# wangxiaohit/GNNPN-SC

Hardware: AMD Instinct MI355X
Metric: service-composition problems/sec (ML+2PN inference) (higher is better)
Workload: dtype f32-split3xf16 (f32 operands and results; recurrent W_hh.h products: fp32 operands split exactly into 3 x f16, six f16-matrix-core products per term, f32 accumulate; everything else f32 arithmetic)

## Files before the change

gnnpn-sc_amd/csrc/api.hip:

```cpp
#include "common.h"
#include <string.h>
#include <mutex>
#include "lstm_shared.h"
#include "decode_shared.h"
#include "coop_common.h"

thread_local char g_gnnpn_err[256] = "";

thread_local int64_t g_gnnpn_last_units = 0;
extern "C" int64_t gnnpn_last_launch_units(void) { return g_gnnpn_last_units; }

thread_local int g_gnnpn_lds_footprint_kb = 0;
extern "C" int gnnpn_lds_footprint_kb(int kb) {
    const int prev = g_gnnpn_lds_footprint_kb;
    if (kb >= 0 && kb <= 160) g_gnnpn_lds_footprint_kb = kb;
    return prev;
}
unsigned gnnpn_front_lds_pad(const void* func) { return gnnpn_lds_padding(func, g_gnnpn_lds_footprint_kb); }

extern "C" int gnnpn_abi_version(void) { return GNNPN_ABI_VERSION; }
extern "C" const char* gnnpn_last_error(void) { return g_gnnpn_err; }

static int g_lstm_ablate = 0;
int gnnpn_option_lstm_ablate() { return g_lstm_ablate; }

unsigned* gnnpn_cu_seat_table() {
    static unsigned* table[64] = {nullptr};
    static std::mutex mu;
    int dev = 0;
    if (hipGetDevice(&dev) != hipSuccess || dev < 0 || dev >= 64) return nullptr;
    std::lock_guard<std::mutex> lock(mu);
    if (!table[dev]) {
        unsigned* p = nullptr;
        if (hipMalloc(&p, COOP_SEAT_TABLE_WORDS * sizeof(unsigned)) != hipSuccess) return nullptr;
        if (hipMemset(p, 0, COOP_SEAT_TABLE_WORDS * sizeof(unsigned)) != hipSuccess) return nullptr;
        if (hipDeviceSynchronize() != hipSuccess) return nullptr;
        table[dev] = p;
    }
    return table[dev];
}

extern "C" int gnnpn_coop_reset_staffing(void) {
    unsigned* p = gnnpn_cu_seat_table();
    if (!p) GNNPN_FAIL(GNNPN_E_LAUNCH, "coop_reset_staffing: no seat table");
    if (hipDeviceSynchronize() != hipSuccess || hipMemset(p + COOP_STAFFING_WORD, 0, sizeof(unsigned)) != hipSuccess)
        GNNPN_FAIL(GNNPN_E_LAUNCH, "coop_reset_staffing: memset failed");
    return GNNPN_OK;
}

extern "C" int gnnpn_coop_staffing_count(void) {
    unsigned* p = gnnpn_cu_seat_table();
    unsigned v = 0;
    if (!p || hipDeviceSynchronize() != hipSuccess || hipMemcpy(&v, p + COOP_STAFFING_WORD, sizeof(v), hipMemcpyDeviceToHost) != hipSuccess) return -1;
    return (int)v;
}

extern "C" int gnnpn_set_option(const char* name, int value) {
    if (!name) GNNPN_FAIL(GNNPN_E_ARG, "set_option: null name");
    if (!strcmp(name, "lstm_ablate")) {
        GNNPN_REQUIRE(value >= 0 && (value & 128) == 0, "set_option: lstm_ablate bit 7 is gnnpn_launch_opts_t.write_through now");
        g_lstm_ablate = value;
        return GNNPN_OK;
    }
    GNNPN_FAIL(GNNPN_E_ARG, "set_option: unknown option '%s' (impl / lds_kb / write_through are gnnpn_launch_opts_t fields)", name);
}

__global__ void cell_activations_kernel(const float* __restrict__ x, float* __restrict__ sig, float* __restrict__ th,
                                        int64_t n) {
    const int64_t i = blockIdx.x * (int64_t)blockDim.x + threadIdx.x;
    if (i < n) {
        sig[i] = cell_sigmoid(x[i]);
        th[i] = cell_tanh(x[i]);
    }
}

extern "C" int gnnpn_debug_cell_activations(const float* x, float* sig, float* th, int64_t n, void* stream) {
    GNNPN_REQUIRE(x && sig && th && n >= 0, "debug_cell_activations: bad argument");
    if (n == 0) return GNNPN_OK;
    hipLaunchKernelGGL(cell_activations_kernel, dim3((unsigned)((n + 255) / 256)), dim3(256), 0, (hipStream_t)stream,
                       x, sig, th, n);
    GNNPN_CHECK_LAUNCH("debug_cell_activations");
    return GNNPN_OK;
}

namespace {
__global__ void gate_wait_kernel(const unsigned* __restrict__ flag, unsigned expect, unsigned long long ticks) {
    const unsigned long long t0 = __builtin_amdgcn_s_memrealtime();
    while (__hip_atomic_load(flag, __ATOMIC_RELAXED, __HIP_MEMORY_SCOPE_SYSTEM) != expect &&
           __builtin_amdgcn_s_memrealtime() - t0 < ticks)
        __builtin_amdgcn_s_sleep(20);
}
}

extern "C" int gnnpn_gate_wait(const void* flag, uint32_t expect, int32_t timeout_us, void* stream) {
    GNNPN_REQUIRE(flag && timeout_us >= 0 && timeout_us <= 100000, "gate_wait: a flag in pinned host (or device) memory, a time-out of at most 0.1 s");
    GNNPN_REQUIRE(gnnpn_aligned(flag, 4), "gate_wait: the flag must be 4-byte aligned");
    hipLaunchKernelGGL(gate_wait_kernel, dim3(1), dim3(64), 0, static_cast<hipStream_t>(stream), static_cast<const unsigned*>(flag), expect,
                       (unsigned long long)timeout_us * 100ull);
    GNNPN_CHECK_LAUNCH("gate_wait");
    return GNNPN_OK;
}
```

gnnpn-sc_amd/csrc/coop_common.h:

```cpp
#pragma once
#include "common.h"
#include "lstm_shared.h"

typedef float f32x4 __attribute__((ext_vector_type(4)));
typedef unsigned long long u64;

__device__ __forceinline__ void granule_store(u64* p, unsigned tag, float v) {
    __hip_atomic_store(p, ((u64)tag << 32) | __float_as_uint(v), __ATOMIC_RELAXED,
                       __HIP_MEMORY_SCOPE_AGENT);
}

typedef unsigned u32x4 __attribute__((ext_vector_type(4)));
#define GNNPN_LD2(dst, voff, sbase, off) "global_load_dwordx4 " dst ", " voff ", " sbase " offset:" off " sc1\n\t"
__device__ __forceinline__ const u64* uniform_ptr(const u64* p) {
    const unsigned long long v = (unsigned long long)p;
    const unsigned lo = __builtin_amdgcn_readfirstlane((unsigned)v), hi = __builtin_amdgcn_readfirstlane((unsigned)(v >> 32));
    return reinterpret_cast<const u64*>(((unsigned long long)hi << 32) | lo);
}
__device__ __forceinline__ void granule_reload2_x8_masked(u32x4 (&v)[8], const u64* base, unsigned voff, unsigned long long lanes) {
    const u64* q = base + 512;
    unsigned long long saved;
    asm volatile("s_and_saveexec_b64 %8, %12\n\t"
                 GNNPN_LD2("%0", "%9", "%10", "0") GNNPN_LD2("%1", "%9", "%10", "1024") GNNPN_LD2("%2", "%9", "%10", "2048")
                 GNNPN_LD2("%3", "%9", "%10", "3072") GNNPN_LD2("%4", "%9", "%11", "0") GNNPN_LD2("%5", "%9", "%11", "1024")
                 GNNPN_LD2("%6", "%9", "%11", "2048") GNNPN_LD2("%7", "%9", "%11", "3072")
                 "s_waitcnt vmcnt(0)\n\t"
                 "s_mov_b64 exec, %8"
                 : "+v"(v[0]), "+v"(v[1]), "+v"(v[2]), "+v"(v[3]), "+v"(v[4]), "+v"(v[5]), "+v"(v[6]), "+v"(v[7]), "=&s"(saved)
                 : "v"(voff), "s"(base), "s"(q), "s"(lanes)
                 : "memory", "scc");
}
__device__ __forceinline__ void granule_load2_x8_x4(u32x4 (&v)[8], u32x4 (&w)[4], const u64* base, const u64* pbase, unsigned voff) {
    const u64* q = base + 512;
    asm volatile(GNNPN_LD2("%0", "%12", "%13", "0") GNNPN_LD2("%1", "%12", "%13", "1024") GNNPN_LD2("%2", "%12", "%13", "2048")
                 GNNPN_LD2("%3", "%12", "%13", "3072") GNNPN_LD2("%4", "%12", "%14", "0") GNNPN_LD2("%5", "%12", "%14", "1024")
                 GNNPN_LD2("%6", "%12", "%14", "2048") GNNPN_LD2("%7", "%12", "%14", "3072")
                 GNNPN_LD2("%8", "%12", "%15", "0") GNNPN_LD2("%9", "%12", "%15", "1024") GNNPN_LD2("%10", "%12", "%15", "2048")
                 GNNPN_LD2("%11", "%12", "%15", "3072")
                 "s_waitcnt vmcnt(0)"
                 : "=&v"(v[0]), "=&v"(v[1]), "=&v"(v[2]), "=&v"(v[3]), "=&v"(v[4]), "=&v"(v[5]), "=&v"(v[6]), "=&v"(v[7]),
                   "=&v"(w[0]), "=&v"(w[1]), "=&v"(w[2]), "=&v"(w[3])
                 : "v"(voff), "s"(base), "s"(q), "s"(pbase)
                 : "memory");
}

__device__ __forceinline__ void granule_load2_x8_x4_lat(u32x4 (&v)[8], u32x4 (&w)[4], u64& lat, const u64* base, const u64* pbase,
                                                        const u64* lbase, unsigned voff) {
    const u64* q = base + 512;
    asm volatile(GNNPN_LD2("%0", "%13", "%15", "0") GNNPN_LD2("%1", "%13", "%15", "1024") GNNPN_LD2("%2", "%13", "%15", "2048")
                 GNNPN_LD2("%3", "%13", "%15", "3072") GNNPN_LD2("%4", "%13", "%16", "0") GNNPN_LD2("%5", "%13", "%16", "1024")
                 GNNPN_LD2("%6", "%13", "%16", "2048") GNNPN_LD2("%7", "%13", "%16", "3072")
                 GNNPN_LD2("%8", "%13", "%17", "0") GNNPN_LD2("%9", "%13", "%17", "1024") GNNPN_LD2("%10", "%13", "%17", "2048")
                 GNNPN_LD2("%11", "%13", "%17", "3072")
                 "global_load_dwordx2 %12, %14, %18 sc1\n\t"
                 "s_waitcnt vmcnt(0)"
                 : "=&v"(v[0]), "=&v"(v[1]), "=&v"(v[2]), "=&v"(v[3]), "=&v"(v[4]), "=&v"(v[5]), "=&v"(v[6]), "=&v"(v[7]),
                   "=&v"(w[0]), "=&v"(w[1]), "=&v"(w[2]), "=&v"(w[3]), "=&v"(lat)
                 : "v"(voff), "v"(voff >> 1), "s"(base), "s"(q), "s"(pbase), "s"(lbase)
                 : "memory");
}

constexpr int COOP_STAFFING_WORD = 8 * 256 + 8;
__device__ __forceinline__ void coop_raise(unsigned* err, unsigned* sticky, unsigned code, unsigned* seats = nullptr) {
    atomicOr(err, code);
    if (sticky) atomicOr(sticky, code);
    if (seats && atomicCAS(err + 4, 1u, 2u) == 1u) atomicSub(seats + COOP_STAFFING_WORD, 1u);
}

constexpr int COOP_STATUS_BYTES = 16384;
constexpr unsigned COOP_LDS_UNITS = 640;
constexpr int COOP_XCD_STRIDE = 32;
constexpr int COOP_XCDCNT_OFFSET = 12288;
constexpr int COOP_ARRIVE_OFFSET = 13312;
constexpr int COOP_PLACED_OFFSET = 14336;
constexpr int COOP_CLAIM_OFFSET = 2048;
constexpr int COOP_TAKEN_OFFSET = 10240;
constexpr int COOP_OVERREAD_BYTES = 4096;
constexpr int COOP_OVERSUB = 3;
constexpr unsigned COOP_SURPLUS_WAIT_TICKS = 1600;
constexpr unsigned COOP_RESERVE_WAIT_TICKS = 200000;

__device__ __forceinline__ unsigned xcc_id() {
    return __builtin_amdgcn_s_getreg(20 | (0 << 6) | (3 << 11)) & 0xfu;
}

__device__ __forceinline__ void granule_store_l2_bits(u64* p, u64 g) {
    asm volatile("global_store_dwordx2 %0, %1, off" ::"v"(p), "v"(g) : "memory");
}
__device__ __forceinline__ void granule_store_l2(u64* p, unsigned tag, float v) {
    granule_store_l2_bits(p, ((u64)tag << 32) | __float_as_uint(v));
}
__device__ __forceinline__ void granule_publish(u64* p, unsigned tag, float v, bool same_xcd) {
    if (same_xcd) granule_store_l2(p, tag, v);
    else granule_store(p, tag, v);
}

namespace {
__global__ __launch_bounds__(256) void coop_zero_kernel(unsigned long long* __restrict__ p, size_t n8, unsigned* __restrict__ sticky,
                                                        int word, unsigned expected, int skip_zeroing) {
    if (sticky && blockIdx.x == 0 && threadIdx.x == 0) atomicAdd(sticky + word, expected);
    if (skip_zeroing) return;
    for (size_t i = blockIdx.x * (size_t)blockDim.x + threadIdx.x; i < n8; i += (size_t)gridDim.x * blockDim.x)
        __hip_atomic_store(p + i, 0ull, __ATOMIC_RELAXED, __HIP_MEMORY_SCOPE_AGENT);
}
}
inline hipError_t coop_zero_workspace(void* workspace, size_t bytes, hipStream_t s, unsigned* sticky, int word, unsigned expected,
                                      bool skip_zeroing = false) {
    const size_t n8 = bytes / 8;
    unsigned blocks = skip_zeroing ? 1u : (unsigned)((n8 + 255) / 256);
    if (blocks > 2048) blocks = 2048;
    hipLaunchKernelGGL(coop_zero_kernel, dim3(blocks), dim3(256), 0, s, static_cast<unsigned long long*>(workspace), n8, sticky, word,
                       expected, skip_zeroing ? 1 : 0);
    return hipGetLastError();
}

constexpr int COOP_G = 8, COOP_ROWS = 16, COOP_H = 256;

struct CoopLaunch {
    int n_tiles, gpx, groups, groups_per_net;
    unsigned* status;
    char* buffers;
    unsigned* seats;
};

template <typename Need>
inline int coop_begin(const char* who, int n_nets, int32_t rows, Need need, int expected_word, const CoopOpts& opts,
                      void* workspace, int64_t workspace_bytes, hipStream_t s, CoopLaunch& L) {
    int dev = 0, n_cu = 0;
    if (hipGetDevice(&dev) != hipSuccess ||
        hipDeviceGetAttribute(&n_cu, hipDeviceAttributeMultiprocessorCount, dev) != hipSuccess)
        GNNPN_FAIL(GNNPN_E_LAUNCH, "%s: cannot query the device", who);
    L.n_tiles = (rows + COOP_ROWS - 1) / COOP_ROWS;
    L.gpx = n_cu / (8 * COOP_G);
    if (L.gpx > 8) L.gpx = 8;
    while (L.gpx > 1 && (L.gpx - 1) * 8 >= n_nets * L.n_tiles) --L.gpx;
    if (L.gpx < 1 || n_cu < 256)
        GNNPN_FAIL(GNNPN_E_UNSUP, "%s: device has %d CUs, the cooperative form is built for 8 XCDs x 32 CUs", who, n_cu);
    L.groups = L.gpx * 8;
    if (L.groups < n_nets) GNNPN_FAIL(GNNPN_E_UNSUP, "%s: %d groups for %d nets", who, L.groups, n_nets);
    L.groups_per_net = L.groups / n_nets;
    const int64_t bytes = need(L.groups);
    if (!workspace || workspace_bytes < bytes || !gnnpn_aligned(workspace, 256))
        GNNPN_FAIL(GNNPN_E_ARG, "%s: workspace of %lld B (256-B aligned) required", who, (long long)bytes);
    L.seats = gnnpn_cu_seat_table();
    if (!L.seats) GNNPN_FAIL(GNNPN_E_LAUNCH, "%s: cannot allocate the seat table", who);
    const unsigned units = (unsigned)(COOP_G * n_nets * L.n_tiles);
    if (coop_zero_workspace(workspace, (size_t)bytes, s, opts.sticky, expected_word, units, (gnnpn_option_lstm_ablate() & 0x2000) != 0) !=
        hipSuccess)
        GNNPN_FAIL(GNNPN_E_LAUNCH, "%s: workspace memset failed", who);
    g_gnnpn_last_units = opts.sticky ? (int64_t)units : 0;
    L.status = static_cast<unsigned*>(workspace);
    L.buffers = static_cast<char*>(workspace) + COOP_STATUS_BYTES;
    return GNNPN_OK;
}

struct DecodeWorkspace {
    int64_t h_bytes, p_bytes, l_bytes;
    int64_t total() const { return COOP_STATUS_BYTES + h_bytes + p_bytes + l_bytes + COOP_OVERREAD_BYTES; }
};
inline DecodeWorkspace decode_workspace(int64_t groups, int64_t rows, int32_t T, int32_t K, int64_t xp_granules) {
    const int64_t tiles = (rows + COOP_ROWS - 1) / COOP_ROWS;
    return {groups * 2 * COOP_ROWS * COOP_H * 8, groups * 2 * xp_granules * 8, tiles * T * COOP_ROWS * (int64_t)K * 8};
}
__device__ __forceinline__ void coop_note_finished(unsigned* sticky, int word, unsigned tiles_done) {
    if (sticky && tiles_done) atomicAdd(sticky + word, tiles_done);
}

__device__ __forceinline__ void coop_note_staffed(unsigned* status, unsigned* count_xcc, unsigned target, unsigned* seats) {
    if (atomicAdd(count_xcc, 1u) + 1u == target && atomicAdd(status + 5, 1u) + 1u == 8u && atomicExch(status + 4, 2u) == 1u)
        atomicSub(seats + COOP_STAFFING_WORD, 1u);
}
template <int G>
__device__ __forceinline__ bool coop_place(unsigned* status, int gpx, int* slot, int& group, int& member, unsigned* seats,
                                           bool paired_start = false, unsigned* sticky = nullptr) {
    if (threadIdx.x < 64) {
        const int lane = threadIdx.x;
        const unsigned xcc = xcc_id();
        unsigned* count = status + COOP_XCDCNT_OFFSET / 4;
        unsigned* arrive = status + COOP_ARRIVE_OFFSET / 4;
        unsigned* taken = status + COOP_TAKEN_OFFSET / 4 + xcc * 64;
        const unsigned target = (unsigned)(gpx * G);
        auto staffed = [&]() {
            unsigned v = 0;
            if (lane == 0) v = __hip_atomic_load(status + 5, __ATOMIC_RELAXED, __HIP_MEMORY_SCOPE_AGENT);
            return __shfl(v, 0, 64) >= 8u;
        };
        int g = -1, m = 0;
#ifndef GNNPN_COOP_NO_ENTRY_ACQUIRE
        __builtin_amdgcn_fence(__ATOMIC_ACQUIRE, "agent");
#endif
        const unsigned hw = __builtin_amdgcn_s_getreg(4 | (0 << 6) | (31 << 11));
        const unsigned key = (xcc << 8) | ((hw >> 8) & 0xffu);
        unsigned* staffing = seats + COOP_STAFFING_WORD;
        const unsigned* word = lane < 8 ? count + COOP_XCD_STRIDE * lane : lane == 9 ? status + 4 : seats + key;
        unsigned got = 0;
        if (lane < 12 && lane != 8 && lane != 10) got = __hip_atomic_load(word, __ATOMIC_RELAXED, __HIP_MEMORY_SCOPE_AGENT);
        if (lane == 8) got = atomicAdd(arrive + COOP_XCD_STRIDE * xcc, 1u);
        const bool staffed_at_entry = __all(lane >= 8 || got >= target);
        unsigned arrival = __shfl(got, 8, 64);
        const bool marked = __shfl(got, 9, 64) != 0u;
        const unsigned seat_seen = __shfl(got, 11, 64);
        if (lane == 0) {
            if (arrival == 0u && !marked && atomicCAS(status + 4, 0u, 1u) == 0u) atomicAdd(staffing, 1u);
            if (arrival >= gridDim.x / 8 || (staffed_at_entry && arrival < target)) coop_raise(status, sticky, 8u);
        }
        if (!staffed_at_entry) {
            if (lane == 0) {
                atomicAdd(status + COOP_CLAIM_OFFSET / 4 + key, 1u);
                const unsigned la = __builtin_amdgcn_s_getreg(6 | (0 << 6) | (31 << 11));
                const unsigned lds_base = la & 0xfffu, lds_size = (la >> 12) & 0xfffu;
                const bool badly_placed = lds_base != 0u && lds_base < lds_size && lds_base + 2u * lds_size > COOP_LDS_UNITS;
                bool another_staffing = false;
                if (badly_placed && !paired_start) {
                    if (atomicCAS(status + 4, 0u, 1u) == 0u) atomicAdd(staffing, 1u);
                    another_staffing = __hip_atomic_load(staffing, __ATOMIC_RELAXED, __HIP_MEMORY_SCOPE_AGENT) > 1u;
                }
                const bool fragments = (paired_start || another_staffing) && badly_placed;
                const bool reserve_arrival = arrival + target >= gridDim.x / 8;
                if (fragments && !reserve_arrival) {
                    atomicAdd(status + 3, 1u);
                    if (sticky) atomicAdd(sticky + GNNPN_STATUS_DECLINED_SEATS, 1u);
                    g = -2;
                } else if (!fragments) {
                    unsigned s = seat_seen;
                    if (s == 0u) {
                        if (atomicCAS(seats + key, 0u, 0xffffffffu) == 0u) {
                            s = atomicAdd(seats + 8 * 256 + xcc, 1u) + 1u;
                            __hip_atomic_store(seats + key, s, __ATOMIC_RELAXED, __HIP_MEMORY_SCOPE_AGENT);
                        } else {
                            s = 0xffffffffu;
                        }
                    }
                    for (unsigned spin = 0; s == 0xffffffffu && spin < 100000u; ++spin)
                        s = __hip_atomic_load(seats + key, __ATOMIC_RELAXED, __HIP_MEMORY_SCOPE_AGENT);
                    const unsigned seat = s - 1u;
                    if (seat < target && atomicCAS(taken + seat, 0u, 1u) == 0u) {
                        g = (int)xcc * gpx + (int)(seat / G);
                        m = (int)(seat % G);
                        coop_note_staffed(status, count + COOP_XCD_STRIDE * xcc, target, seats);
                    }
                }
            }
            g = __shfl(g, 0, 64);
            m = __shfl(m, 0, 64);
            arrival = __shfl(arrival, 0, 64);
            if (g == -2) {
                g = -1;
            } else if (g < 0) {
                const unsigned per_xcd = gridDim.x / 8;
                const bool reserve = arrival + target >= per_xcd;
                const unsigned long long patience = reserve ? COOP_RESERVE_WAIT_TICKS : COOP_SURPLUS_WAIT_TICKS;
                const unsigned long long t0 = __builtin_amdgcn_s_memrealtime();
                bool done = staffed();
                while (!done && __builtin_amdgcn_s_memrealtime() - t0 < patience) {
                    __builtin_amdgcn_s_sleep(8);
                    done = staffed();
                }
                if (!done && reserve) {
                    if (lane == 0) {
                        for (unsigned seat = 0; seat < target && g < 0; ++seat) {
                            if (atomicCAS(taken + seat, 0u, 1u) == 0u) {
                                g = (int)xcc * gpx + (int)(seat / G);
                                m = (int)(seat % G);
                                coop_note_staffed(status, count + COOP_XCD_STRIDE * xcc, target, seats);
                                atomicAdd(status + 2, 1u);
                                if (sticky) atomicAdd(sticky + GNNPN_STATUS_OFF_CANONICAL_SEATS, 1u);
                            }
                        }
                    }
                    g = __shfl(g, 0, 64);
                    m = __shfl(m, 0, 64);
                }
            }
        }
        if (lane == 0) {
            slot[0] = g;
            slot[1] = m;
        }
    }
    __syncthreads();
    group = slot[0];
    member = slot[1];
    return group >= 0;
}

__device__ __forceinline__ float swap8(float v) {
    return __int_as_float(__builtin_amdgcn_update_dpp(0, __float_as_int(v), 0x128 , 0xF, 0xF, false));
}

__device__ __forceinline__ u64 phase_stamp() {
    u64 t;
    __builtin_amdgcn_sched_barrier(0);
    asm volatile("s_memtime %0\n\ts_waitcnt lgkmcnt(0)" : "=s"(t)::"memory");
    __builtin_amdgcn_sched_barrier(0);
    return t;
}

constexpr int LDT = 260;
__device__ __forceinline__ int ht_index(int row, int unit) { return row * LDT + (unit & 3) * 64 + (unit >> 2); }

struct NoHook {
    __device__ __forceinline__ void operator()() const {}
};
template <int LD, int CH = 16, bool KQ = false, typename Mid = NoHook>
__device__ __forceinline__ void mfma_chain_pair(const float* src, int c, int kq, const float (&w0)[64],
                                                const float (&w1)[64], f32x4& acc0, f32x4& acc1, Mid mid = Mid()) {
    const float* base = KQ ? src + c * LD + kq * 64 : src + c * LD + kq;
    const float4* base4 = reinterpret_cast<const float4*>(base);
    float a[2][CH];
    auto fetch = [&](int ch, float (&dst)[CH]) {
        if constexpr (KQ) {
#pragma unroll
            for (int q = 0; q < CH / 4; ++q) {
                const float4 v = base4[(CH / 4) * ch + q];
                dst[4 * q] = v.x; dst[4 * q + 1] = v.y; dst[4 * q + 2] = v.z; dst[4 * q + 3] = v.w;
            }
        } else {
#pragma unroll
            for (int i = 0; i < CH; ++i) dst[i] = base[4 * (CH * ch + i)];
        }
    };
    fetch(0, a[0]);
#pragma unroll
    for (int ch = 0; ch < 64 / CH; ++ch) {
        if (ch < 64 / CH - 1) fetch(ch + 1, a[(ch + 1) & 1]);
        __builtin_amdgcn_sched_barrier(0);
#pragma unroll
        for (int i = 0; i < CH; ++i) {
            acc0 = __builtin_amdgcn_mfma_f32_16x16x4f32(a[ch & 1][i], w0[CH * ch + i], acc0, 0, 0, 0);
            acc1 = __builtin_amdgcn_mfma_f32_16x16x4f32(a[ch & 1][i], w1[CH * ch + i], acc1, 0, 0, 0);
        }
        __builtin_amdgcn_sched_barrier(0);
        if (ch == 64 / CH / 2 - 1) mid();
    }
}

typedef _Float16 f16x8 __attribute__((ext_vector_type(8)));
constexpr int LDH16 = 264;
constexpr int SPLIT_TILE = 16 * LDH16;
constexpr float SPLIT_SCALE = 2048.0f, SPLIT_INV = 1.0f / 2048.0f;
constexpr float SPLIT_H_SCALE = 32768.0f, SPLIT_H_INV = 1.0f / 32768.0f;

__device__ __forceinline__ void split3(float xs, _Float16& p0, _Float16& p1, _Float16& p2) {
    p0 = (_Float16)xs;
    const float r1 = __fmul_rn(__fsub_rn(xs, (float)p0), SPLIT_SCALE);
    p1 = (_Float16)r1;
    p2 = (_Float16)__fmul_rn(__fsub_rn(r1, (float)p1), SPLIT_SCALE);
}
__device__ __forceinline__ unsigned short f16_bits(_Float16 v) { return __builtin_bit_cast(unsigned short, v); }

__device__ __forceinline__ unsigned split_tag16(unsigned tag) { return 0x8000u | (tag & 0x7fffu); }
__device__ __forceinline__ u64 split_granule(unsigned tag, float h) {
    _Float16 p0, p1, p2;
    split3(__fmul_rn(h, SPLIT_H_SCALE), p0, p1, p2);
    const unsigned d0 = (unsigned)f16_bits(p0) | (split_tag16(tag) << 16);
    const unsigned d1 = (unsigned)f16_bits(p1) | ((unsigned)f16_bits(p2) << 16);
    return ((u64)d1 << 32) | d0;
}
__device__ __forceinline__ void split_granule_store(u64* p, unsigned tag, float h, bool same_xcd) {
    const u64 g = split_granule(tag, h);
    if (same_xcd) granule_store_l2_bits(p, g);
    else __hip_atomic_store(p, g, __ATOMIC_RELAXED, __HIP_MEMORY_SCOPE_AGENT);
}
__device__ __forceinline__ bool split_pair_tagged(u32x4 v, unsigned tag) {
    const unsigned t = split_tag16(tag);
    return __builtin_amdgcn_perm(v.z, v.x, 0x07060302u) == (t | (t << 16));
}
__device__ __forceinline__ void split_pair_to_lds(_Float16* at, u32x4 v) {
    unsigned* d = reinterpret_cast<unsigned*>(at);
    d[0] = __builtin_amdgcn_perm(v.z, v.x, 0x05040100u);
    d[SPLIT_TILE / 2] = __builtin_amdgcn_perm(v.w, v.y, 0x05040100u);
    d[SPLIT_TILE] = __builtin_amdgcn_perm(v.w, v.y, 0x07060302u);
}
__device__ __forceinline__ void split_store(_Float16* at, float h) {
    _Float16 p0, p1, p2;
    split3(__fmul_rn(h, SPLIT_H_SCALE), p0, p1, p2);
    at[0] = p0;
    at[SPLIT_TILE] = p1;
    at[2 * SPLIT_TILE] = p2;
}

constexpr int SPLIT_WT_DWORDS = 4 * 8 * 64 * 4;
template <int HD>
__device__ __forceinline__ float split_weights(const float* __restrict__ Wp, int gate, int u, int kq, f16x8 (&w0)[8],
                                               f16x8 (&w1)[8], unsigned* wt) {
    float m = 0.0f;
#pragma unroll
    for (int kk = 0; kk < 8; ++kk)
#pragma unroll
        for (int j = 0; j < 8; ++j)
            m = fmaxf(m, fabsf(Wp[((size_t)((8 * kk + 2 * kq + (j >> 2)) * 4 + gate) * HD + u) * 4 + (j & 3)]));
    m = fmaxf(m, __shfl_xor(m, 16, 64));
    m = fmaxf(m, __shfl_xor(m, 32, 64));
    int e = 0;
    if (m > 0.0f && m < 3.0e38f) (void)frexpf(m, &e);
    int s = m > 0.0f ? 15 - e : 0;
    s = s > 96 ? 96 : (s < -96 ? -96 : s);
    const float up = ldexpf(1.0f, s);
#pragma unroll
    for (int kk = 0; kk < 8; ++kk) {
        unsigned bytes[2] = {0u, 0u};
#pragma unroll
        for (int j = 0; j < 8; ++j) {
            const float w = Wp[((size_t)((8 * kk + 2 * kq + (j >> 2)) * 4 + gate) * HD + u) * 4 + (j & 3)];
            _Float16 p0, p1, p2;
            split3(__fmul_rn(w, up), p0, p1, p2);
            w0[kk][j] = p0;
            w1[kk][j] = p1;
            bytes[j >> 2] |= (unsigned)(f16_bits(p2) >> 8) << (8 * (j & 3));
        }
        wt[4 * 64 * kk] = bytes[0];
        wt[4 * 64 * kk + 1] = bytes[1];
    }
    return ldexpf(1.0f, -(15 + s));
}
constexpr int SPLIT_PACK_U4_PER_MEMBER = 2 * 2 * 8 * 256 + 8 * 256 + 2 * 256 / 4;
constexpr int SPLIT_PACK_MEMBERS = 8;
__device__ __forceinline__ void load_split_weights(const uint4* __restrict__ pk, int tid, f16x8 (&w0)[2][8], f16x8 (&w1)[2][8],
                                                   unsigned* wt_lane, float (&inv)[2]) {
#pragma unroll
    for (int tl = 0; tl < 2; ++tl)
#pragma unroll
        for (int kk = 0; kk < 8; ++kk) {
            w0[tl][kk] = __builtin_bit_cast(f16x8, pk[((tl * 2 + 0) * 8 + kk) * 256 + tid]);
            w1[tl][kk] = __builtin_bit_cast(f16x8, pk[((tl * 2 + 1) * 8 + kk) * 256 + tid]);
        }
#pragma unroll
    for (int kk = 0; kk < 8; ++kk) *reinterpret_cast<uint4*>(wt_lane + 4 * 64 * kk) = pk[8192 + kk * 256 + tid];
    const float* fi = reinterpret_cast<const float*>(pk + 10240);
    inv[0] = fi[tid];
    inv[1] = fi[256 + tid];
}

__device__ __forceinline__ f16x8 split_expand(unsigned lo, unsigned hi) {
    const u32x4 r = {__builtin_amdgcn_perm(0u, lo, 0x010c000cu), __builtin_amdgcn_perm(0u, lo, 0x030c020cu),
                     __builtin_amdgcn_perm(0u, hi, 0x010c000cu), __builtin_amdgcn_perm(0u, hi, 0x030c020cu)};
    return __builtin_bit_cast(f16x8, r);
}
template <typename Mid = NoHook>
__device__ __forceinline__ void split_chain(const _Float16* base, const f16x8 (&w0)[2][8], const f16x8 (&w1)[2][8],
                                            const unsigned* wt, const float (&inv)[2], f32x4 (&acc)[2], Mid mid = Mid()) {
    constexpr int NT = 2;
    f32x4 a0[NT], a0b[NT], a1[NT], a2[NT];
#pragma unroll
    for (int n = 0; n < NT; ++n) a0[n] = a0b[n] = a1[n] = a2[n] = f32x4{0.f, 0.f, 0.f, 0.f};
    f16x8 h0[2];
    h0[0] = *reinterpret_cast<const f16x8*>(base);
    f16x8 h1 = *reinterpret_cast<const f16x8*>(base + SPLIT_TILE);
    f16x8 h2 = *reinterpret_cast<const f16x8*>(base + 2 * SPLIT_TILE);
    u32x4 t = *reinterpret_cast<const u32x4*>(wt);
#define GNNPN_FENCE __builtin_amdgcn_sched_barrier(0)
#pragma unroll
    for (int kk = 0; kk < 8; ++kk) {
        const int nx = 32 * (kk + 1), cur = kk & 1;
        u32x4 e0, e1;
        if (kk < 7) h0[cur ^ 1] = *reinterpret_cast<const f16x8*>(base + nx);
        GNNPN_FENCE;
        a2[0] = __builtin_amdgcn_mfma_f32_16x16x32_f16(h1, w1[0][kk], a2[0], 0, 0, 0);
        e0.x = __builtin_amdgcn_perm(0u, t.x, 0x010c000cu);
        e0.y = __builtin_amdgcn_perm(0u, t.x, 0x030c020cu);
        GNNPN_FENCE;
        a2[1] = __builtin_amdgcn_mfma_f32_16x16x32_f16(h1, w1[1][kk], a2[1], 0, 0, 0);
        e0.z = __builtin_amdgcn_perm(0u, t.y, 0x010c000cu);
        e0.w = __builtin_amdgcn_perm(0u, t.y, 0x030c020cu);
        GNNPN_FENCE;
        a1[0] = __builtin_amdgcn_mfma_f32_16x16x32_f16(h1, w0[0][kk], a1[0], 0, 0, 0);
        e1.x = __builtin_amdgcn_perm(0u, t.z, 0x010c000cu);
        e1.y = __builtin_amdgcn_perm(0u, t.z, 0x030c020cu);
        GNNPN_FENCE;
        a1[1] = __builtin_amdgcn_mfma_f32_16x16x32_f16(h1, w0[1][kk], a1[1], 0, 0, 0);
        e1.z = __builtin_amdgcn_perm(0u, t.w, 0x010c000cu);
        e1.w = __builtin_amdgcn_perm(0u, t.w, 0x030c020cu);
        GNNPN_FENCE;
        if (kk < 7) {
            h1 = *reinterpret_cast<const f16x8*>(base + SPLIT_TILE + nx);
            t = *reinterpret_cast<const u32x4*>(wt + 4 * 64 * (kk + 1));
        }
        a2[0] = __builtin_amdgcn_mfma_f32_16x16x32_f16(h0[cur], __builtin_bit_cast(f16x8, e0), a2[0], 0, 0, 0);
        GNNPN_FENCE;
        a2[1] = __builtin_amdgcn_mfma_f32_16x16x32_f16(h0[cur], __builtin_bit_cast(f16x8, e1), a2[1], 0, 0, 0);
        GNNPN_FENCE;
        if (kk < 4) a0[0] = __builtin_amdgcn_mfma_f32_16x16x32_f16(h0[cur], w0[0][kk], a0[0], 0, 0, 0);
        else a0b[0] = __builtin_amdgcn_mfma_f32_16x16x32_f16(h0[cur], w0[0][kk], a0b[0], 0, 0, 0);
        GNNPN_FENCE;
        if (kk < 4) a0[1] = __builtin_amdgcn_mfma_f32_16x16x32_f16(h0[cur], w0[1][kk], a0[1], 0, 0, 0);
        else a0b[1] = __builtin_amdgcn_mfma_f32_16x16x32_f16(h0[cur], w0[1][kk], a0b[1], 0, 0, 0);
        GNNPN_FENCE;
        a2[0] = __builtin_amdgcn_mfma_f32_16x16x32_f16(h2, w0[0][kk], a2[0], 0, 0, 0);
        GNNPN_FENCE;
        a2[1] = __builtin_amdgcn_mfma_f32_16x16x32_f16(h2, w0[1][kk], a2[1], 0, 0, 0);
        GNNPN_FENCE;
        if (kk < 7) h2 = *reinterpret_cast<const f16x8*>(base + 2 * SPLIT_TILE + nx);
        a1[0] = __builtin_amdgcn_mfma_f32_16x16x32_f16(h0[cur], w1[0][kk], a1[0], 0, 0, 0);
        GNNPN_FENCE;
        a1[1] = __builtin_amdgcn_mfma_f32_16x16x32_f16(h0[cur], w1[1][kk], a1[1], 0, 0, 0);
        GNNPN_FENCE;
        if (kk == 3) mid();
    }
#undef GNNPN_FENCE
#pragma unroll
    for (int n = 0; n < NT; ++n)
#pragma unroll
        for (int r = 0; r < 4; ++r)
            acc[n][r] = __fmul_rn(fmaf(fmaf(a2[n][r], SPLIT_INV, a1[n][r]), SPLIT_INV, __fadd_rn(a0[n][r], a0b[n][r])), inv[n]);
}

__device__ __forceinline__ void cell_update_split(const f32x2 (&g0)[2], const f32x2 (&g1)[2], bool lo_half, f32x2& cst, f32x2& h) {
    f32x2 a0[2], a1[2];
#pragma unroll
    for (int q = 0; q < 2; ++q) {
        a0[q] = cell_act2(g0[q], false);
        a1[q] = cell_act2(g1[q], lo_half);
    }
    const f32x2 s0 = lo_half ? a0[1] : a0[0], s1 = lo_half ? a1[1] : a1[0];
    const f32x2 t0 = {swap8(s0.x), swap8(s0.y)}, t1 = {swap8(s1.x), swap8(s1.y)};
    const f32x2 ig = lo_half ? a0[0] : t0, gg = lo_half ? a1[0] : t1;
    const f32x2 fg = lo_half ? t0 : a0[1], og = lo_half ? t1 : a1[1];
    cst = fg * cst + ig * gg;
    h = og * cell_act2(cst, true);
}
```

gnnpn-sc_amd/csrc/decode_lean.hip:

```cpp
#include "common.h"
#include "recurrent.h"
#include "decode_shared.h"
#include "coop_common.h"
#include "lstm_shared.h"

namespace {
constexpr int H = COOP_H;
constexpr int G = COOP_G;
constexpr int ROWS = COOP_ROWS;
constexpr int UNITS = H / G;
constexpr int KW = 16;
constexpr unsigned SPIN_LIMIT = 400000;
constexpr int XP_GRANULES = ROWS * KW * G;

typedef unsigned u32x2 __attribute__((ext_vector_type(2)));
constexpr int AUX_SC1 = 16;


__device__ __forceinline__ __amdgpu_buffer_rsrc_t make_rsrc(const void* p, unsigned bytes) {
    return __builtin_amdgcn_make_buffer_rsrc(const_cast<void*>(p), 0, (int)bytes, 0x00020000);
}
__device__ __forceinline__ float dpp_ror(float v, int n) {
    switch (n) {
        case 1: return __int_as_float(__builtin_amdgcn_update_dpp(0, __float_as_int(v), 0x121, 0xF, 0xF, true));
        case 2: return __int_as_float(__builtin_amdgcn_update_dpp(0, __float_as_int(v), 0x122, 0xF, 0xF, true));
        case 4: return __int_as_float(__builtin_amdgcn_update_dpp(0, __float_as_int(v), 0x124, 0xF, 0xF, true));
        default: return __int_as_float(__builtin_amdgcn_update_dpp(0, __float_as_int(v), 0x128, 0xF, 0xF, true));
    }
}
__device__ __forceinline__ void store_granule(__amdgpu_buffer_rsrc_t r, unsigned voff, unsigned soff, u64 g, bool same_xcd) {
    const u32x2 v = {(unsigned)g, (unsigned)(g >> 32)};
    if (same_xcd) __builtin_amdgcn_raw_buffer_store_b64(v, r, voff, soff, 0);
    else __builtin_amdgcn_raw_buffer_store_b64(v, r, voff, soff, AUX_SC1);
}
__device__ __forceinline__ void record_failure(unsigned* diag, const unsigned* err, int group, int member, int tile, int k, int wave,
                                               unsigned tag, unsigned h_miss, unsigned p_miss, unsigned l_miss, int gpx) {
    if ((threadIdx.x & 63) != 0 || !diag) return;
    const unsigned n = atomicAdd(diag, 1u);
    if (n >= 31) return;
    unsigned* rec = diag + 16 * (n + 1);
    const unsigned* cnt = err + COOP_XCDCNT_OFFSET / 4;
    unsigned c0 = 0, c1 = 0;
    for (int x = 0; x < 4; ++x) {
        c0 |= (cnt[COOP_XCD_STRIDE * x] & 0xffu) << (8 * x);
        c1 |= (cnt[COOP_XCD_STRIDE * (4 + x)] & 0xffu) << (8 * x);
    }
    const unsigned long long t = __builtin_amdgcn_s_memrealtime();
    rec[0] = group; rec[1] = member; rec[2] = tile; rec[3] = k; rec[4] = wave; rec[5] = tag;
    rec[6] = h_miss; rec[7] = p_miss; rec[8] = l_miss; rec[9] = c0; rec[10] = c1;
    rec[11] = (unsigned)t; rec[12] = (unsigned)(t >> 32); rec[13] = gpx; rec[14] = blockIdx.x; rec[15] = err[0];
}
}

template <bool SPLIT, int OCC, int EVH, bool DIAG = false>
__global__ __launch_bounds__(256, OCC) void pointer_decode_lean_kernel(DecodeArgs a, u64* xh, u64* xp,
                                                                     u64* xl, unsigned* __restrict__ err,
                                                                     unsigned* __restrict__ sticky, int n_nets, int groups_per_net,
                                                                     int gpx, int write_through, unsigned* __restrict__ seats,
                                                                     unsigned* __restrict__ diag) {
    __shared__ __attribute__((aligned(16))) float hs[SPLIT ? 3 * SPLIT_TILE / 2 : ROWS * LDT];
    __shared__ __attribute__((aligned(16))) unsigned wts[SPLIT ? SPLIT_WT_DWORDS : 4];
    __shared__ __attribute__((aligned(16))) float hsl[ROWS][UNITS + 4];
    __shared__ __attribute__((aligned(16))) float win[ROWS][KW][8];
    __shared__ int sel[ROWS];
    __shared__ int abort_flag;
    __shared__ int place[2];

    const int tid = threadIdx.x, lane = tid & 63, wave = __builtin_amdgcn_readfirstlane(tid >> 6);
    const int kq = lane >> 4, c = lane & 15;
    int group, member;
    if (!coop_place<G>(err, gpx, place, group, member, seats, (write_through & 2) != 0, sticky)) return;
    group = __builtin_amdgcn_readfirstlane(group);
    member = __builtin_amdgcn_readfirstlane(member);
    const int net_id = group / groups_per_net, gi = group % groups_per_net;
    if (net_id >= n_nets) return;
    const DecodeNet& net = a.net[net_id];
    if (tid == 0) abort_flag = 0;
    __syncthreads();
    const bool same_xcd = !(write_through & 1);
    if (tid == 0 && same_xcd) atomicAdd(err + COOP_PLACED_OFFSET / 4 + COOP_XCD_STRIDE * xcc_id(), 1u);

    const int B = a.B, T = a.T, K = a.K, L = T * K;
    const bool latent_in_launch = net.latent_from >= 0;
    const bool has_lat = latent_in_launch || net.latent_win;
    bool publishes_latent = false;
    for (int n = 0; n < n_nets; ++n) publishes_latent |= (a.net[n].latent_from == net_id);
    const bool first = member == 0;

    const int unit = member * UNITS + wave * 8 + (c & 7);
    const int wrow0 = (0 + (c >> 3)) * H + unit, wrow1 = (2 + (c >> 3)) * H + unit;
    float wBh[SPLIT ? 1 : 2][SPLIT ? 1 : 64];
    f16x8 wH16[SPLIT ? 2 : 1][8], wL16[SPLIT ? 2 : 1][8];
    float winv[2] = {1.0f, 1.0f};
    unsigned* wt_lane = wts + (SPLIT ? (wave * 8 * 64 + lane) * 4 : 0);
    float bh[2], bi[2], sg[2], wXf[2][2];
    const uint4* __restrict__ Wsplit = SPLIT ? static_cast<const uint4*>(net.whh_split) : nullptr;
    if constexpr (SPLIT) {
        if (Wsplit) load_split_weights(Wsplit + (size_t)member * SPLIT_PACK_U4_PER_MEMBER, tid, wH16, wL16, wt_lane, winv);
    }
#pragma unroll
    for (int tl = 0; tl < 2; ++tl) {
        const int wrow = tl ? wrow1 : wrow0, gate = wrow / H, u = wrow % H;
        bh[tl] = net.bhh[wrow];
        if constexpr (SPLIT) {
            if (!Wsplit) winv[tl] = split_weights<H>(net.whh, gate, u, kq, wH16[tl], wL16[tl], wt_lane + 2 * tl);
        } else {
#pragma unroll
            for (int kk = 0; kk < 64; ++kk) wBh[tl][kk] = net.whh[((size_t)(kk * 4 + gate) * H + u) * 4 + kq];
        }
        wXf[tl][0] = net.xw_fold[wrow * 8 + kq];
        wXf[tl][1] = net.xw_fold[wrow * 8 + 4 + kq];
        bi[tl] = net.xb_fold[wrow];
        sg[tl] = net.start_fold[wrow];
    }

    const int own0 = kq * 4 + (c < 8 ? 0 : 2);
    const int vo_hpub = (int)(own0 * H + unit) * 8u;
    const int vo_sweep = 16 * lane;
    constexpr int VO_NONE = (int)0xFFFFFF00u;
    const int rq = kq, r = c;
    const bool live = r < K;
    const int vo_p = live ? 64 * lane : VO_NONE;
    const int vo_lat = live ? (int)(rq * K + r) * 8u : VO_NONE;
    const int vo_wl = (int)((wave * 4 + rq) * T * K + r) * 4u;
    const int vo_idx = (int)((wave * 4 + rq) * T) * 4u;
    const int vo_act = (int)(c * T * 8 + kq) * 4u;
    const int vo_q = (int)(own0 * T * H + unit) * 4u;
    constexpr int EVN = 8 / EVH;
    const int ppair = tid / EVH, phalf = tid - ppair * EVH;
    const int prow = ppair / K, pcand = ppair - prow * K;
    const bool pdot = ppair < ROWS * K;
    const int vo_ev = pdot ? (int)(((size_t)prow * L + pcand) * H + member * UNITS + phalf * (4 * EVN)) * 4u : VO_NONE;
    const int vo_ppub = (int)((prow * KW + pcand) * G + member) * 8u;
    const int wr_row = tid >> 4, wr_cand = tid & 15;
    const bool wr_live = wr_cand < K;
    const int vo_win = wr_live ? (int)(((size_t)wr_row * L + wr_cand) * 8) * 4u : VO_NONE;

    __amdgpu_buffer_rsrc_t r_h = make_rsrc(xh + (size_t)group * (2 * ROWS * H), 2 * ROWS * H * 8);
    __amdgpu_buffer_rsrc_t r_p = make_rsrc(xp + (size_t)group * (2 * XP_GRANULES), 2 * XP_GRANULES * 8);

    const int n_tiles = (B + ROWS - 1) / ROWS;
    unsigned step = 0;
    unsigned tiles_done = 0;
    for (int tile = gi; tile < n_tiles; tile += groups_per_net) {
        const int b0 = tile * ROWS;
        const int rows_here = min(ROWS, B - b0);
        __amdgpu_buffer_rsrc_t r_enc = make_rsrc(net.enc_out + (size_t)b0 * L * H, (unsigned)((size_t)rows_here * L * H * 4));
        __amdgpu_buffer_rsrc_t r_in = make_rsrc(a.inputs + (size_t)b0 * L * 8, (unsigned)((size_t)rows_here * L * 32));
        __amdgpu_buffer_rsrc_t r_lat = make_rsrc(xl + (size_t)tile * T * ROWS * K, (unsigned)((size_t)T * ROWS * K * 8));
        __amdgpu_buffer_rsrc_t r_wl = make_rsrc(net.win_logits + (size_t)b0 * T * K, (unsigned)((size_t)rows_here * T * K * 4));
        __amdgpu_buffer_rsrc_t r_idx = make_rsrc(net.idx + (size_t)b0 * T, (unsigned)((size_t)rows_here * T * 4));
        __amdgpu_buffer_rsrc_t r_act = make_rsrc(net.actions + (size_t)b0 * T * 8, (unsigned)((size_t)rows_here * T * 32));
        __amdgpu_buffer_rsrc_t r_lw = make_rsrc(net.latent_win ? net.latent_win + (size_t)b0 * T * K : nullptr,
                                                net.latent_win ? (unsigned)((size_t)rows_here * T * K * 4) : 0u);
        __amdgpu_buffer_rsrc_t r_q = make_rsrc(net.queries ? net.queries + (size_t)b0 * T * H : nullptr,
                                               net.queries ? (unsigned)((size_t)rows_here * T * H * 4) : 0u);
        f32x2 cst, hl = {0.f, 0.f};
        cst.x = b0 + own0 < B ? net.c0[(int64_t)(b0 + own0) * H + unit] : 0.0f;
        cst.y = b0 + own0 + 1 < B ? net.c0[(int64_t)(b0 + own0 + 1) * H + unit] : 0.0f;
        __syncthreads();
        for (int j = 0; j < ROWS; ++j) {
            const float h0v = (b0 + j < B) ? net.h0[(int64_t)(b0 + j) * H + tid] : 0.0f;
            if constexpr (SPLIT) split_store(reinterpret_cast<_Float16*>(hs) + j * LDH16 + tid, h0v);
            else hs[ht_index(j, tid)] = h0v;
        }
        __syncthreads();

        for (int k = 0; k <= T; ++k) {
            float axf0 = 0.0f, axf1 = 0.0f;
            u64 st[8] = {0, 0, 0, 0, 0, 0, 0, 0};
            if constexpr (DIAG) st[0] = st[1] = st[2] = st[3] = st[4] = st[5] = phase_stamp();
            const unsigned tag = step;
            const unsigned par = (step - 1) & 1;
            const unsigned so_k = (unsigned)k * (unsigned)K;
            u32x4 ev[EVN];
            u32x4 vp[4];
            u32x2 vl;
#pragma unroll
            for (int j = 0; j < EVN; ++j) asm volatile("" : "=v"(ev[j]));
#pragma unroll
            for (int j = 0; j < 4; ++j) asm volatile("" : "=v"(vp[j]));
            asm volatile("" : "=v"(vl));
            f32x4 ah[2] = {f32x4{0.f, 0.f, 0.f, 0.f}, f32x4{0.f, 0.f, 0.f, 0.f}};

            constexpr bool EV_EARLY = OCC == 1;
            auto request_ev = [&]() {
#pragma unroll
                for (int j = 0; j < EVN; ++j) ev[j] = __builtin_amdgcn_raw_buffer_load_b128(r_enc, vo_ev, so_k * (H * 4) + 16u * j, 0);
            };
            if (k < T) {
                if (k > 0) {
                    const unsigned so_h0 = par * (ROWS * H * 8) + wave * (4 * H * 8);
                    u32x4 vh[8];
                    bool ok = false;
                    unsigned h_miss = 0;
                    for (unsigned spins = 0; spins <= SPIN_LIMIT; ++spins) {
                        unsigned so_h = so_h0;
                        asm volatile("" : "+s"(so_h));
#pragma unroll
                        for (int j = 0; j < 8; ++j) vh[j] = __builtin_amdgcn_raw_buffer_load_b128(r_h, vo_sweep, so_h + 1024u * j, AUX_SC1);
                        bool good = true;
#pragma unroll
                        for (int j = 0; j < 8; ++j) {
                            if constexpr (SPLIT) good &= split_pair_tagged(vh[j], tag);
                            else good &= (vh[j].y == tag) & (vh[j].w == tag);
                        }
                        if (__all(good)) {
                            ok = true;
                            break;
                        }
                        __builtin_amdgcn_s_sleep(1);
                    }
                    if constexpr (DIAG) st[1] = phase_stamp();
                    if (!ok) {
                        abort_flag = 1;
#pragma unroll
                        for (int j = 0; j < 8; ++j) {
                            bool bad;
                            if constexpr (SPLIT) bad = !split_pair_tagged(vh[j], tag);
                            else bad = (vh[j].y != tag) | (vh[j].w != tag);
                            const unsigned long long bm = __ballot(bad);
                            for (int q = 0; q < 4; ++q)
                                if ((bm >> (16 * q)) & 0xffffull) h_miss |= 1u << (4 * (j & 1) + q);
                        }
                        record_failure(diag, err, group, member, tile, k, wave, tag, h_miss, 0u, 0u, gpx);
                    }
#pragma unroll
                    for (int j = 0; j < 8; ++j) {
                        const int i = 2 * (j * 64 + lane);
                        if constexpr (SPLIT) {
                            split_pair_to_lds(reinterpret_cast<_Float16*>(hs) + (wave * 4 + (i >> 8)) * LDH16 + (i & 255), vh[j]);
                        } else {
                            float* d = &hs[ht_index(wave * 4 + (i >> 8), i & 255)];
                            d[0] = __uint_as_float(vh[j].x);
                            d[64] = __uint_as_float(vh[j].z);
                        }
                    }
                    if constexpr (EV_EARLY) request_ev();
                    __syncthreads();
                    if (abort_flag) break;
                } else if constexpr (EV_EARLY) {
                    request_ev();
                }
                if constexpr (DIAG) st[2] = phase_stamp();
                constexpr bool EARLY_P = OCC == 1 || !SPLIT;
                auto request_p = [&]() {
                    if (EARLY_P && k > 0) {
                        const unsigned so_p = par * (XP_GRANULES * 8) + wave * (4 * KW * G * 8);
#pragma unroll
                        for (int j = 0; j < 4; ++j) vp[j] = __builtin_amdgcn_raw_buffer_load_b128(r_p, vo_p, so_p + 16u * j, AUX_SC1);
                        if (latent_in_launch)
                            vl = __builtin_amdgcn_raw_buffer_load_b64(r_lat, vo_lat, (unsigned)(((k - 1) * ROWS + wave * 4) * K) * 8u, AUX_SC1);
                    }
                };
                if constexpr (SPLIT) split_chain(reinterpret_cast<const _Float16*>(hs) + c * LDH16 + 8 * kq, wH16, wL16, wt_lane, winv, ah, request_p);
                else mfma_chain_pair<LDT, OCC == 2 ? 8 : 16, true>(hs, c, kq, wBh[0], wBh[SPLIT ? 0 : 1], ah[0], ah[1], request_p);
                if constexpr (DIAG) {
                    asm volatile("" ::"v"(ah[0][0]), "v"(ah[1][0]));
                    st[3] = phase_stamp();
                }
            }

            if (k > 0) {
                const unsigned so_p0 = par * (XP_GRANULES * 8) + wave * (4 * KW * G * 8);
                const unsigned so_l0 = (unsigned)(((k - 1) * ROWS + wave * 4) * K) * 8u;
                bool ok = false;
                for (unsigned spins = 0; spins <= SPIN_LIMIT; ++spins) {
                    if (spins > 0 || k == T || (OCC != 1 && SPLIT)) {
                        unsigned so_p = so_p0, so_l = so_l0;
                        asm volatile("" : "+s"(so_p), "+s"(so_l));
#pragma unroll
                        for (int j = 0; j < 4; ++j) vp[j] = __builtin_amdgcn_raw_buffer_load_b128(r_p, vo_p, so_p + 16u * j, AUX_SC1);
                        if (latent_in_launch) vl = __builtin_amdgcn_raw_buffer_load_b64(r_lat, vo_lat, so_l, AUX_SC1);
                    }
                    bool good = true;
                    if (live) {
#pragma unroll
                        for (int j = 0; j < 4; ++j) good &= (vp[j].y == tag) & (vp[j].w == tag);
                        if (latent_in_launch) good &= vl.y == 1u;
                    }
                    if (__all(good)) {
                        ok = true;
                        break;
                    }
                    __builtin_amdgcn_s_sleep(1);
                }
                if constexpr (DIAG) st[4] = phase_stamp();
                if (!ok) {
                    abort_flag = 1;
                    unsigned p_miss = 0;
#pragma unroll
                    for (int j = 0; j < 4; ++j) {
                        if (__ballot(live && vp[j].y != tag)) p_miss |= 1u << (2 * j);
                        if (__ballot(live && vp[j].w != tag)) p_miss |= 1u << (2 * j + 1);
                    }
                    record_failure(diag, err, group, member, tile, k, wave, tag, 0u, p_miss, (unsigned)__popcll(__ballot(live && latent_in_launch && vl.y != 1u)), gpx);
                }

                {
                    const int row = wave * 4 + rq;
                    const unsigned so_t = (unsigned)(k - 1) * (unsigned)K * 4u;
                    float dot = 0.0f, lv = 0.0f;
                    if (live) {
                        dot = __fadd_rn(__fadd_rn(__fadd_rn(__uint_as_float(vp[0].x), __uint_as_float(vp[0].z)), __uint_as_float(vp[1].x)), __uint_as_float(vp[1].z));
                        dot = __fadd_rn(__fadd_rn(__fadd_rn(__fadd_rn(dot, __uint_as_float(vp[2].x)), __uint_as_float(vp[2].z)), __uint_as_float(vp[3].x)), __uint_as_float(vp[3].z));
                        if (latent_in_launch) lv = __uint_as_float(vl.x);
                        else if (net.latent_win) lv = __uint_as_float(__builtin_amdgcn_raw_buffer_load_b32(r_lw, vo_wl, so_t, 0));
                    }
                    float v = a.use_tanh ? __fmul_rn(a.tanh_c, tanhf(dot)) : dot;
                    if (live && first) {
                        __builtin_amdgcn_raw_buffer_store_b32(__float_as_uint(v), r_wl, vo_wl, so_t, 0);
                        if (publishes_latent)
                            __builtin_amdgcn_raw_buffer_store_b64(u32x2{__float_as_uint(v), 1u}, r_lat, vo_lat, so_l0, AUX_SC1);
                    }
                    v = (has_lat && live) ? __fadd_rn(v, lv) : v;
                    float m = live ? v : -INFINITY;
                    m = fmaxf(m, dpp_ror(m, 8));
                    m = fmaxf(m, dpp_ror(m, 4));
                    m = fmaxf(m, dpp_ror(m, 2));
                    m = fmaxf(m, dpp_ror(m, 1));
                    const unsigned hit = (unsigned)(__ballot(live && v == m) >> (16 * rq)) & 0xffffu;
                    const int pick_r = hit ? __ffs(hit) - 1 : 0;
                    if (r == 0) {
                        sel[row] = pick_r;
                        if (first) __builtin_amdgcn_raw_buffer_store_b32((unsigned)((k - 1) * K + pick_r), r_idx, vo_idx, (unsigned)(k - 1) * 4u, 0);
                    }
                }
                __syncthreads();
                if (abort_flag) break;
                axf0 = win[c][sel[c]][kq];
                axf1 = win[c][sel[c]][4 + kq];
                if (first && wave == 0) {
                    __builtin_amdgcn_raw_buffer_store_b32(__float_as_uint(axf0), r_act, vo_act, (unsigned)(k - 1) * 32u, 0);
                    __builtin_amdgcn_raw_buffer_store_b32(__float_as_uint(axf1), r_act, vo_act, (unsigned)(k - 1) * 32u + 16u, 0);
                }
                if (k == T) break;
                if constexpr (DIAG) st[5] = phase_stamp();
            }

            if constexpr (!EV_EARLY) request_ev();
            u32x4 wv0, wv1;
            wv0 = __builtin_amdgcn_raw_buffer_load_b128(r_in, vo_win, so_k * 32u, 0);
            wv1 = __builtin_amdgcn_raw_buffer_load_b128(r_in, vo_win, so_k * 32u + 16u, 0);
            float gx[2][4];
            if (k > 0) {
                f32x4 ax0 = {0.f, 0.f, 0.f, 0.f}, ax1 = ax0;
                ax0 = __builtin_amdgcn_mfma_f32_16x16x4f32(axf0, wXf[0][0], ax0, 0, 0, 0);
                ax1 = __builtin_amdgcn_mfma_f32_16x16x4f32(axf0, wXf[1][0], ax1, 0, 0, 0);
                ax0 = __builtin_amdgcn_mfma_f32_16x16x4f32(axf1, wXf[0][1], ax0, 0, 0, 0);
                ax1 = __builtin_amdgcn_mfma_f32_16x16x4f32(axf1, wXf[1][1], ax1, 0, 0, 0);
#pragma unroll
                for (int q = 0; q < 4; ++q) {
                    gx[0][q] = __fadd_rn(ax0[q], bi[0]);
                    gx[1][q] = __fadd_rn(ax1[q], bi[1]);
                }
            } else {
#pragma unroll
                for (int q = 0; q < 4; ++q) {
                    gx[0][q] = sg[0];
                    gx[1][q] = sg[1];
                }
            }
            {
                f32x2 g0[2], g1[2];
#pragma unroll
                for (int q = 0; q < 2; ++q) {
                    g0[q] = (f32x2{ah[0][2 * q], ah[0][2 * q + 1]} + pk_set(bh[0])) + f32x2{gx[0][2 * q], gx[0][2 * q + 1]};
                    g1[q] = (f32x2{ah[1][2 * q], ah[1][2 * q + 1]} + pk_set(bh[1])) + f32x2{gx[1][2 * q], gx[1][2 * q + 1]};
                }
                cell_update_split(g0, g1, c < 8, cst, hl);
            }
            {
                const unsigned so_pub = (step & 1) * (ROWS * H * 8);
                if constexpr (SPLIT) {
                    store_granule(r_h, vo_hpub, so_pub, split_granule(step + 1, hl.x), same_xcd);
                    store_granule(r_h, vo_hpub, so_pub + H * 8, split_granule(step + 1, hl.y), same_xcd);
                } else {
                    store_granule(r_h, vo_hpub, so_pub, ((u64)(step + 1) << 32) | __float_as_uint(hl.x), same_xcd);
                    store_granule(r_h, vo_hpub, so_pub + H * 8, ((u64)(step + 1) << 32) | __float_as_uint(hl.y), same_xcd);
                }
                hsl[own0][wave * 8 + (c & 7)] = hl.x;
                hsl[own0 + 1][wave * 8 + (c & 7)] = hl.y;
                if (net.queries) {
                    __builtin_amdgcn_raw_buffer_store_b32(__float_as_uint(hl.x), r_q, vo_q, (unsigned)k * (H * 4), 0);
                    __builtin_amdgcn_raw_buffer_store_b32(__float_as_uint(hl.y), r_q, vo_q, (unsigned)(k + T) * (H * 4), 0);
                }
            }
            if constexpr (DIAG) {
                asm volatile("" ::"v"(hl.y));
                st[6] = phase_stamp();
            }
            __syncthreads();
            {
                float p = 0.0f;
                if (pdot) {
#pragma unroll
                    for (int j = 0; j < EVN; ++j) {
                        const float4 hv = *reinterpret_cast<const float4*>(&hsl[prow][phalf * (4 * EVN) + 4 * j]);
                        p = fmaf(__uint_as_float(ev[j].x), hv.x, p);
                        p = fmaf(__uint_as_float(ev[j].y), hv.y, p);
                        p = fmaf(__uint_as_float(ev[j].z), hv.z, p);
                        p = fmaf(__uint_as_float(ev[j].w), hv.w, p);
                    }
                }
                if constexpr (EVH == 2)
                    p = __fadd_rn(p, __int_as_float(__builtin_amdgcn_update_dpp(0, __float_as_int(p), 0xB1 , 0xF, 0xF, false)));
                if (pdot && phalf == 0)
                    store_granule(r_p, vo_ppub, (step & 1) * (XP_GRANULES * 8), ((u64)(step + 1) << 32) | __float_as_uint(p), same_xcd);
            }
            if (wr_live) {
                *reinterpret_cast<u32x4*>(&win[wr_row][wr_cand][0]) = wv0;
                *reinterpret_cast<u32x4*>(&win[wr_row][wr_cand][4]) = wv1;
            }
            if constexpr (DIAG) {
                st[7] = phase_stamp();
                if (blockIdx.x == 0 && tid == 0 && k > 0) {
                    u64* prof = reinterpret_cast<u64*>(err) + 4;
                    prof[0] += st[1] - st[0];
                    prof[1] += st[2] - st[1];
                    prof[2] += st[3] - st[2];
                    prof[3] += st[4] - st[3];
                    prof[4] += st[5] - st[4];
                    prof[5] += st[6] - st[5];
                    prof[6] += st[7] - st[6];
                    prof[7] += 1;
                }
            }
            ++step;
        }
        if (abort_flag) break;
        ++tiles_done;
    }
    if (tid == 0) {
        if (abort_flag) coop_raise(err, sticky, 2u, seats);
        coop_note_finished(sticky, GNNPN_STATUS_DEC_FINISHED, tiles_done);
    }
}

struct PickProbArgs {
    const float* win[2];
    const float* lat[2];
    const int32_t* idx[2];
    float* out[2];
};
__global__ __launch_bounds__(256) void pick_prob_kernel(PickProbArgs a, int64_t rows, int T, int K) {
    const int net = blockIdx.y;
    const float* __restrict__ win = a.win[net];
    const float* __restrict__ lat = a.lat[net];
    const int32_t* __restrict__ idx = a.idx[net];
    float* __restrict__ out = a.out[net];
    const int64_t row = blockIdx.x * 256ll + threadIdx.x;
    if (row >= rows) return;
    const unsigned t_base = (unsigned)__builtin_amdgcn_readfirstlane((int)((blockIdx.x * 256ll) % T));
    const int t = (int)((t_base + threadIdx.x) % (unsigned)T);
    float v[16];
#pragma unroll
    for (int j = 0; j < 16; ++j) {
        v[j] = 0.0f;
        if (j < K) {
            v[j] = win[row * K + j];
            if (lat) v[j] = __fadd_rn(v[j], lat[row * K + j]);
        }
    }
    const int pick_r = min(max(idx[row] - t * K, 0), 15);
    float best = v[0];
#pragma unroll
    for (int j = 1; j < 16; ++j) best = j == pick_r ? v[j] : best;
#pragma unroll
    for (int j = 0; j < 16; ++j) v[j] = j < K ? expf(__fsub_rn(v[j], best)) : 0.0f;
#pragma unroll
    for (int n = 8; n >= 1; n >>= 1)
#pragma unroll
        for (int j = 0; j < n; ++j) v[j] = __fadd_rn(v[j], v[j + n]);
    out[row] = 1.0f / v[0];
}

static DecodeWorkspace lean_workspace(int64_t groups, int64_t rows, int32_t T, int32_t K) {
    return decode_workspace(groups, rows, T, K, XP_GRANULES);
}

int64_t gnnpn_decode_lean_workspace_bytes(int32_t B, int32_t T, int32_t n_per) { return lean_workspace(64, B, T, n_per).total(); }

int gnnpn_launch_decode_lean(const DecodeArgs& args, int n_nets, int precision, bool shared_cu, const CoopOpts& opts,
                             void* workspace, int64_t workspace_bytes, hipStream_t s) {
    if (args.K > KW) GNNPN_FAIL(GNNPN_E_UNSUP, "pointer_decode: the cooperative form is built for n_per <= %d", KW);
    if ((int64_t)ROWS * args.T * args.K * H * 4 >= (1ll << 32) || (int64_t)args.T * ROWS * args.K * 8 >= (1ll << 32))
        GNNPN_FAIL(GNNPN_E_UNSUP, "pointer_decode: a tile of 16 problems must stay below 4 GB of encoder output");
    const bool split = precision == GNNPN_PREC_SPLIT;
    const bool wide = args.K > 8;
    const bool stamps = (gnnpn_option_lstm_ablate() & 0x800) != 0;
    if (stamps && wide) GNNPN_FAIL(GNNPN_E_UNSUP, "pointer_decode: the stamped build exists for n_per <= 8");
    CoopLaunch c;
    const auto need = [&](int groups) { return lean_workspace(groups, args.B, args.T, args.K).total(); };
    if (const int rc = coop_begin("pointer_decode", n_nets, args.B, need, GNNPN_STATUS_DEC_EXPECTED, opts, workspace, workspace_bytes, s, c))
        return rc;
    const DecodeWorkspace w = lean_workspace(c.groups, args.B, args.T, args.K);
    u64* p_h = reinterpret_cast<u64*>(c.buffers);
    u64* p_p = reinterpret_cast<u64*>(c.buffers + w.h_bytes);
    u64* p_l = reinterpret_cast<u64*>(c.buffers + w.h_bytes + w.p_bytes);
    static unsigned* p_diag = gnnpn_decode_diag_buffer();
    const int wt = (opts.write_through ? 1 : 0) | (opts.paired_start ? 2 : 0);
#define GNNPN_LEAN(SPLIT_, OCC_, EVH_, ...)                                                                                           \
    hipLaunchKernelGGL((pointer_decode_lean_kernel<SPLIT_, OCC_, EVH_, ##__VA_ARGS__>), dim3(COOP_OVERSUB * c.groups * G), dim3(256),       \
                       gnnpn_lds_padding((const void*)pointer_decode_lean_kernel<SPLIT_, OCC_, EVH_, ##__VA_ARGS__>, opts.lds_kb), s, args, \
                       p_h, p_p, p_l, c.status, opts.sticky, n_nets, c.groups_per_net, c.gpx, wt, c.seats, p_diag)
    if (stamps) {
        if (split) GNNPN_LEAN(true, 1, 2, true);
        else GNNPN_LEAN(false, 1, 2, true);
    } else if (split && shared_cu && wide) GNNPN_LEAN(true, 2, 1);
    else if (split && shared_cu) GNNPN_LEAN(true, 2, 2);
    else if (split && wide) GNNPN_LEAN(true, 1, 1);
    else if (split) GNNPN_LEAN(true, 1, 2);
    else if (shared_cu && wide) GNNPN_LEAN(false, 2, 1);
    else if (shared_cu) GNNPN_LEAN(false, 2, 2);
    else if (wide) GNNPN_LEAN(false, 1, 1);
    else GNNPN_LEAN(false, 1, 2);
#undef GNNPN_LEAN
    if (hipGetLastError() != hipSuccess) GNNPN_FAIL(GNNPN_E_LAUNCH, "pointer_decode: launch of the cooperative kernel failed");
    const int64_t rows = (int64_t)args.B * args.T;
    for (int n0 = 0; n0 < n_nets; n0 += 2) {
        PickProbArgs pa = {};
        const int cnt = n_nets - n0 < 2 ? n_nets - n0 : 2;
        for (int n = 0; n < cnt; ++n) {
            const DecodeNet& d = args.net[n0 + n];
            pa.win[n] = d.win_logits;
            pa.lat[n] = d.latent_from >= 0 ? args.net[d.latent_from].win_logits : d.latent_win;
            pa.idx[n] = d.idx;
            pa.out[n] = d.pick_prob;
        }
        hipLaunchKernelGGL(pick_prob_kernel, dim3((unsigned)((rows + 255) / 256), (unsigned)cnt), dim3(256), 0, s, pa, rows, args.T, args.K);
    }
    return GNNPN_OK;
}
```

gnnpn-sc_amd/csrc/lstm_coop.hip:

```cpp
#include "common.h"
#include "recurrent.h"
#include "lstm_shared.h"
#include "coop_common.h"
#include "decode_shared.h"

namespace {
constexpr int H = COOP_H;
constexpr int G = COOP_G;
constexpr int ROWS = COOP_ROWS;
constexpr int UNITS = H / G;
constexpr unsigned SPIN_LIMIT = 400000;
constexpr int GROUP_GRANULES = 2 * ROWS * H + 2 * 4 * G;
constexpr int ENC_LOOP_PAD_NOPS = 13;
}

template <int PREC>
__device__ __forceinline__ bool sweep_quarter(const u64* buf, unsigned tag, float* hs, int wave, int lane, bool keep,
                                              bool nowait = false) {
    const u64* src = uniform_ptr(buf + wave * 4 * H);
    const unsigned voff = 16u * lane;
    u32x4 v[8];
#pragma unroll
    for (int j = 0; j < 8; ++j) asm volatile("" : "=v"(v[j]));
    bool bad = true;
    unsigned spins = 0;
    int nap = 1;
    for (;;) {
        granule_reload2_x8_masked(v, src, voff, __ballot(bad));
        bad = false;
#pragma unroll
        for (int j = 0; j < 8; ++j) {
            if constexpr (PREC == 2) bad |= !split_pair_tagged(v[j], tag);
            else bad |= (v[j].y != tag) | (v[j].w != tag);
        }
        if (!__any(bad) || nowait) break;
        if (++spins > SPIN_LIMIT) return false;
        for (int z = 0; z < nap; ++z) __builtin_amdgcn_s_sleep(2);
        if (nap < 16) nap <<= 1;
    }
    if (keep) {
#pragma unroll
        for (int j = 0; j < 8; ++j) {
            const int i = 2 * (j * 64 + lane);
            if constexpr (PREC == 0) {
                float* d = &hs[ht_index(wave * 4 + (i >> 8), i & 255)];
                d[0] = __uint_as_float(v[j].x);
                d[64] = __uint_as_float(v[j].z);
            } else {
                _Float16* h16 = reinterpret_cast<_Float16*>(hs) + (wave * 4 + (i >> 8)) * LDH16 + (i & 255);
                if constexpr (PREC == 2) {
                    split_pair_to_lds(h16, v[j]);
                } else {
                    h16[0] = (_Float16)__uint_as_float(v[j].x);
                    h16[1] = (_Float16)__uint_as_float(v[j].z);
                }
            }
        }
    }
    return true;
}


template <int PREC, bool PRE, bool DIAG>
__global__ __launch_bounds__(256, 2) void lstm_encode_coop_kernel(LstmNets nets, u64* __restrict__ xchg,
                                                                  unsigned* __restrict__ err, unsigned* __restrict__ sticky,
                                                                  int32_t B, int32_t L, int n_nets, int groups_per_net,
                                                                  int gpx, int ablate_arg, unsigned* __restrict__ seats,
                                                                  unsigned* __restrict__ diag) {
    const int ablate = DIAG ? (ablate_arg & ~0x1000) : (ablate_arg & 128);
    constexpr bool F16 = PREC != 0, SPLIT = PREC == 2;
    constexpr int HS_FLOATS = PREC == 2 ? 3 * SPLIT_TILE / 2 : ROWS * LDH16;
    __shared__ __attribute__((aligned(16))) float hs[HS_FLOATS];
    __shared__ __attribute__((aligned(16))) float hst[ROWS][UNITS];
    __shared__ int abort_flag;

    const int lane = threadIdx.x & 63, wave = threadIdx.x >> 6;
    const int kq = lane >> 4, c = lane & 15;
    __shared__ int place[2];
    int group, member;
    u64 p_entry = 0, p_placed = 0, p_weights = 0;
    if constexpr (DIAG) p_entry = phase_stamp();
    if (!coop_place<G>(err, gpx, place, group, member, seats, (ablate_arg & 0x1000) != 0, sticky)) return;
    if constexpr (DIAG) p_placed = phase_stamp();
    const int net = group / groups_per_net, gi = group % groups_per_net;
    if (net >= n_nets) return;
    if (threadIdx.x == 0) abort_flag = 0;
    __syncthreads();
    const bool same_xcd = !(ablate & 128);
    if (threadIdx.x == 0 && same_xcd) atomicAdd(err + COOP_PLACED_OFFSET / 4 + COOP_XCD_STRIDE * xcc_id(), 1u);

    const float* __restrict__ pre = PRE ? nets.pregates[net] : nullptr;
    const float* __restrict__ xin = nets.inputs[net];
    const float* __restrict__ Wp = nets.whh[net];
    float* __restrict__ enc = nets.enc_out[net];
    u64* xg = xchg + (size_t)group * GROUP_GRANULES;

    const int unit = member * UNITS + wave * 8 + (c & 7);
    int wrow[2];
    wrow[0] = (0 + (c >> 3)) * H + unit;
    wrow[1] = (2 + (c >> 3)) * H + unit;
    float wB[F16 ? 1 : 2][F16 ? 1 : 64], bh[2], wX[2][2] = {{0.f, 0.f}, {0.f, 0.f}}, bx[2] = {0.f, 0.f};
    f16x8 wB16[F16 ? 2 : 1][8];
    f16x8 wL16[SPLIT ? 2 : 1][8];
    float winv[2] = {1.0f, 1.0f};
    __shared__ __attribute__((aligned(16))) unsigned wts[SPLIT ? SPLIT_WT_DWORDS : 4];
    unsigned* wt_lane = wts + (SPLIT ? (wave * 8 * 64 + lane) * 4 : 0);
    const uint4* __restrict__ Wsplit = SPLIT ? static_cast<const uint4*>(nets.whh_split[net]) : nullptr;
    if constexpr (SPLIT) {
        if (Wsplit) load_split_weights(Wsplit + (size_t)member * SPLIT_PACK_U4_PER_MEMBER, threadIdx.x, wB16, wL16, wt_lane, winv);
    }
#pragma unroll
    for (int tl = 0; tl < 2; ++tl) {
        const int gate = wrow[tl] / H, u = wrow[tl] % H;
        bh[tl] = nets.bhh[net][wrow[tl]];
        if constexpr (SPLIT) {
            if (!Wsplit) winv[tl] = split_weights<H>(Wp, gate, u, kq, wB16[tl], wL16[tl], wt_lane + 2 * tl);
        } else if constexpr (F16) {
#pragma unroll
            for (int kk = 0; kk < 8; ++kk)
#pragma unroll
                for (int j = 0; j < 8; ++j)
                    wB16[tl][kk][j] = (_Float16)Wp[((size_t)((8 * kk + 2 * kq + (j >> 2)) * 4 + gate) * H + u) * 4 + (j & 3)];
        }
        if constexpr (!PRE) {
            wX[tl][0] = nets.w_in[net][wrow[tl] * 8 + kq];
            wX[tl][1] = nets.w_in[net][wrow[tl] * 8 + 4 + kq];
            bx[tl] = nets.b_in[net][wrow[tl]];
        }
        if constexpr (!F16) {
#pragma unroll
            for (int kk = 0; kk < 64; ++kk)
                wB[tl][kk] = Wp[((size_t)(kk * 4 + gate) * H + u) * 4 + kq];
        }
    }

    if constexpr (DIAG) {
        asm volatile("" ::"v"(winv[0]), "v"(winv[1]), "v"(bh[0]), "v"(bh[1]));
        p_weights = phase_stamp();
    }
    const int n_tiles = (B + ROWS - 1) / ROWS;
    unsigned step = 0;
    unsigned tiles_done = 0;
    bool first_tile = true;
    for (int tile = gi; tile < n_tiles; tile += groups_per_net) {
        const int b0 = tile * ROWS;
        f32x2 cst = {0.f, 0.f};
        f32x2 hlast = {0.f, 0.f};
        float pg[2][4], pg_next[2][4] = {{0.f, 0.f, 0.f, 0.f}, {0.f, 0.f, 0.f, 0.f}};
        float ax[2] = {0.f, 0.f}, ax_next[2] = {0.f, 0.f};
        auto load_input = [&](int t, float (&pgv)[2][4], float (&axv)[2]) {
            if constexpr (PRE) {
#pragma unroll
                for (int r = 0; r < 4; ++r) {
                    const int b = b0 + kq * 4 + r;
#pragma unroll
                    for (int tl = 0; tl < 2; ++tl)
                        pgv[tl][r] = b < B ? pre[((int64_t)b * L + t) * (4 * H) + wrow[tl]] : 0.0f;
                }
            } else if (b0 + c < B) {
                const float* row = xin + ((int64_t)(b0 + c) * L + t) * 8;
                axv[0] = row[kq];
                axv[1] = row[4 + kq];
            }
        };
        load_input(0, pg_next, ax_next);
#ifndef GNNPN_ENC_PAD_NOPS
#define GNNPN_ENC_PAD_NOPS ENC_LOOP_PAD_NOPS
#endif
        if constexpr (SPLIT && !DIAG) asm volatile(".p2align 6\n\t.rept %0\n\ts_nop 0\n\t.endr" ::"n"(GNNPN_ENC_PAD_NOPS) : "memory");
        for (int t = 0; t < L; ++t, ++step) {
            const bool stamps = ablate & 32;
            u64 s0 = 0, s1 = 0, s2 = 0, s3 = 0, s4 = 0, s5 = 0;
            if (stamps) s0 = phase_stamp();
#pragma unroll
            for (int tl = 0; tl < 2; ++tl) {
                ax[tl] = ax_next[tl];
#pragma unroll
                for (int r = 0; r < 4; ++r) pg[tl][r] = pg_next[tl][r];
            }
            f32x4 px0 = {0.f, 0.f, 0.f, 0.f}, px1 = {0.f, 0.f, 0.f, 0.f};
            if constexpr (!PRE) {
                px0 = __builtin_amdgcn_mfma_f32_16x16x4f32(ax[0], wX[0][0], px0, 0, 0, 0);
                px1 = __builtin_amdgcn_mfma_f32_16x16x4f32(ax[0], wX[1][0], px1, 0, 0, 0);
                px0 = __builtin_amdgcn_mfma_f32_16x16x4f32(ax[1], wX[0][1], px0, 0, 0, 0);
                px1 = __builtin_amdgcn_mfma_f32_16x16x4f32(ax[1], wX[1][1], px1, 0, 0, 0);
            }
            bool ok = true;
            if (t == 0) {
                for (int i = threadIdx.x; i < HS_FLOATS; i += 256) hs[i] = 0.0f;
                if (!first_tile) ok = sweep_quarter<PREC>(xg + ((step - 1) & 1) * (ROWS * H), step, hs, wave, lane, false);
            } else if (!(ablate & 8)) {
                ok = sweep_quarter<PREC>(xg + ((step - 1) & 1) * (ROWS * H), step, hs, wave, lane, true, ablate & 4);
            }
            if (!ok) abort_flag = 1;
            if constexpr (DIAG) {
                if (!ok && lane == 0 && diag) {
                    const unsigned n = atomicAdd(diag, 1u);
                    if (n < 31) {
                        unsigned* rec = diag + 16 * (n + 1);
                        const unsigned* cnt = err + COOP_XCDCNT_OFFSET / 4;
                        const unsigned* arr = err + COOP_ARRIVE_OFFSET / 4;
                        unsigned c0 = 0, c1 = 0, a0 = 0, a1 = 0;
                        for (int x = 0; x < 4; ++x) {
                            c0 |= (cnt[COOP_XCD_STRIDE * x] & 0xffu) << (8 * x);
                            c1 |= (cnt[COOP_XCD_STRIDE * (4 + x)] & 0xffu) << (8 * x);
                            a0 |= (arr[COOP_XCD_STRIDE * x] & 0xffu) << (8 * x);
                            a1 |= (arr[COOP_XCD_STRIDE * (4 + x)] & 0xffu) << (8 * x);
                        }
                        rec[0] = group; rec[1] = member; rec[2] = tile; rec[3] = t; rec[4] = wave; rec[5] = step;
                        rec[6] = 0; rec[7] = 0xE0Cu; rec[8] = 0; rec[9] = c0; rec[10] = c1; rec[11] = a0; rec[12] = a1;
                        rec[13] = gpx; rec[14] = blockIdx.x; rec[15] = err[0];
                    }
                }
            }
            if (stamps) s1 = phase_stamp();
            __syncthreads();
            if (abort_flag) break;
            if (stamps) s2 = phase_stamp();
            f32x4 acc0 = {0.f, 0.f, 0.f, 0.f}, acc1 = {0.f, 0.f, 0.f, 0.f};
            u64 s2a = 0;
            if (stamps) s2a = phase_stamp();
            if constexpr (SPLIT) {
                if (t > 0) {
                    f32x4 acc[2] = {acc0, acc1};
                    split_chain(reinterpret_cast<const _Float16*>(hs) + c * LDH16 + 8 * kq, wB16, wL16, wt_lane, winv, acc);
                    acc0 = acc[0];
                    acc1 = acc[1];
                }
            } else if constexpr (F16) {
                if (t > 0) {
                    const _Float16* base = reinterpret_cast<const _Float16*>(hs) + c * LDH16 + 8 * kq;
                    f16x8 a16[8];
#pragma unroll
                    for (int kk = 0; kk < 8; ++kk) a16[kk] = *reinterpret_cast<const f16x8*>(base + 32 * kk);
#pragma unroll
                    for (int kk = 0; kk < 8; ++kk) {
                        acc0 = __builtin_amdgcn_mfma_f32_16x16x32_f16(a16[kk], wB16[0][kk], acc0, 0, 0, 0);
                        acc1 = __builtin_amdgcn_mfma_f32_16x16x32_f16(a16[kk], wB16[1][kk], acc1, 0, 0, 0);
                    }
                }
            } else {
                if (t > 0 && !(ablate & 1)) mfma_chain_pair<LDT, 16, true>(hs, c, kq, wB[0], wB[F16 ? 0 : 1], acc0, acc1);
            }
            if (t + 1 < L && !(ablate & 0x400)) load_input(t + 1, pg_next, ax_next);
            if (t > 0 && threadIdx.x < ROWS * 8 && !(ablate & 0x200)) {
                const int row = threadIdx.x >> 3, q = threadIdx.x & 7;
                if (b0 + row < B)
                    *reinterpret_cast<float4*>(enc + ((int64_t)(b0 + row) * L + (t - 1)) * H + member * UNITS + 4 * q) =
                        *reinterpret_cast<const float4*>(&hst[row][4 * q]);
            }

            if (stamps) {
                asm volatile("" ::"v"(acc0[0]), "v"(acc1[0]));
                s3 = phase_stamp();
            }
            if constexpr (!PRE) {
#pragma unroll
                for (int r = 0; r < 4; ++r) {
                    pg[0][r] = __fadd_rn(px0[r], bx[0]);
                    pg[1][r] = __fadd_rn(px1[r], bx[1]);
                }
            }
            __syncthreads();
            if (stamps) s4 = phase_stamp();

            u64* out_buf = xg + (step & 1) * (ROWS * H);
            {
                f32x2 g0[2], g1[2];
#pragma unroll
                for (int q = 0; q < 2; ++q) {
                    g0[q] = (f32x2{acc0[2 * q], acc0[2 * q + 1]} + pk_set(bh[0])) + f32x2{pg[0][2 * q], pg[0][2 * q + 1]};
                    g1[q] = (f32x2{acc1[2 * q], acc1[2 * q + 1]} + pk_set(bh[1])) + f32x2{pg[1][2 * q], pg[1][2 * q + 1]};
                }
                cell_update_split(g0, g1, c < 8, cst, hlast);
            }
            {
                const int r0 = kq * 4 + (c < 8 ? 0 : 2);
                u64* dst = out_buf + r0 * H + unit;
                if constexpr (SPLIT) {
                    split_granule_store(dst, step + 1, hlast.x, same_xcd);
                    split_granule_store(dst + H, step + 1, hlast.y, same_xcd);
                } else if (!(ablate & 16)) {
                    if (same_xcd) {
                        granule_store_l2(dst, step + 1, hlast.x);
                        granule_store_l2(dst + H, step + 1, hlast.y);
                    } else {
                        granule_store(dst, step + 1, hlast.x);
                        granule_store(dst + H, step + 1, hlast.y);
                    }
                }
                hst[r0][wave * 8 + (c & 7)] = hlast.x;
                hst[r0 + 1][wave * 8 + (c & 7)] = hlast.y;
            }
            if (stamps) {
                asm volatile("" ::"v"(hlast.y));
                s5 = phase_stamp();
                if (blockIdx.x == 0 && threadIdx.x == 0 && t > 0) {
                    u64* prof = reinterpret_cast<u64*>(err) + 4;
                    prof[0] += s1 - s0;
                    prof[1] += s2 - s1;
                    prof[2] += s3 - s2;
                    prof[6] += s2a - s2;
                    prof[3] += s4 - s3;
                    prof[4] += s5 - s4;
                    prof[5] += 1;
                    if (t == 1 && first_tile) {
                        prof[7] = p_placed - p_entry;
                        prof[8] = p_weights - p_placed;
                        prof[9] = s0 - p_weights;
                    }
                }
            }
        }
        if (abort_flag) break;
        __syncthreads();
        if (threadIdx.x < ROWS * 8) {
            const int row = threadIdx.x >> 3, q = threadIdx.x & 7;
            if (b0 + row < B)
                *reinterpret_cast<float4*>(enc + ((int64_t)(b0 + row) * L + (L - 1)) * H + member * UNITS + 4 * q) =
                    *reinterpret_cast<const float4*>(&hst[row][4 * q]);
        }
#pragma unroll
        for (int r = 0; r < 2; ++r) {
            const int b = b0 + kq * 4 + (c < 8 ? 0 : 2) + r;
            if (b < B) {
                nets.h_n[net][(int64_t)b * H + unit] = r ? hlast.y : hlast.x;
                nets.c_n[net][(int64_t)b * H + unit] = r ? cst.y : cst.x;
            }
        }
        first_tile = false;
        ++tiles_done;
    }
    if (threadIdx.x == 0) {
        if (abort_flag) coop_raise(err, sticky, 1u, seats);
        coop_note_finished(sticky, GNNPN_STATUS_ENC_FINISHED, tiles_done);
    }
}


__global__ __launch_bounds__(256) void lstm_pack_split_kernel(const float* __restrict__ Wp, uint4* __restrict__ out) {
    __shared__ __attribute__((aligned(16))) unsigned wts[SPLIT_WT_DWORDS];
    const int tid = threadIdx.x, lane = tid & 63, wave = tid >> 6, kq = lane >> 4, c = lane & 15;
    const int member = blockIdx.x;
    const int unit = member * UNITS + wave * 8 + (c & 7);
    f16x8 w0[2][8], w1[2][8];
    float inv[2];
    unsigned* wt_lane = wts + (wave * 8 * 64 + lane) * 4;
#pragma unroll
    for (int tl = 0; tl < 2; ++tl) inv[tl] = split_weights<H>(Wp, 2 * tl + (c >> 3), unit, kq, w0[tl], w1[tl], wt_lane + 2 * tl);
    uint4* pk = out + (size_t)member * SPLIT_PACK_U4_PER_MEMBER;
#pragma unroll
    for (int tl = 0; tl < 2; ++tl)
#pragma unroll
        for (int kk = 0; kk < 8; ++kk) {
            pk[((tl * 2 + 0) * 8 + kk) * 256 + tid] = __builtin_bit_cast(uint4, w0[tl][kk]);
            pk[((tl * 2 + 1) * 8 + kk) * 256 + tid] = __builtin_bit_cast(uint4, w1[tl][kk]);
        }
#pragma unroll
    for (int kk = 0; kk < 8; ++kk) pk[8192 + kk * 256 + tid] = *reinterpret_cast<const uint4*>(wt_lane + 4 * 64 * kk);
    float* fi = reinterpret_cast<float*>(pk + 10240);
    fi[tid] = inv[0];
    fi[256 + tid] = inv[1];
}

extern "C" int64_t gnnpn_lstm_split_weights_bytes(void) { return (int64_t)SPLIT_PACK_MEMBERS * SPLIT_PACK_U4_PER_MEMBER * 16; }

extern "C" int gnnpn_lstm_pack_split_weights_f32(const float* whh_packed, void* split, void* stream) {
    GNNPN_REQUIRE(whh_packed && split, "lstm_pack_split_weights: null operand");
    GNNPN_REQUIRE(gnnpn_aligned(whh_packed, 16) && gnnpn_aligned(split, 16), "lstm_pack_split_weights: operands must be 16-byte aligned");
    static_assert(G == SPLIT_PACK_MEMBERS, "one packed block per group member");
    hipLaunchKernelGGL(lstm_pack_split_kernel, dim3(G), dim3(256), 0, (hipStream_t)stream, whh_packed, static_cast<uint4*>(split));
    GNNPN_CHECK_LAUNCH("lstm_pack_split_weights");
    return GNNPN_OK;
}

static int64_t encode_workspace_bytes(int groups) { return COOP_STATUS_BYTES + (int64_t)groups * GROUP_GRANULES * sizeof(u64); }

extern "C" int64_t gnnpn_lstm_encode_workspace_bytes(void) {
    (void)gnnpn_cu_seat_table();
    return encode_workspace_bytes(64);
}

int gnnpn_launch_encode_coop(const LstmNets& nets, int n_nets, int32_t B, int32_t L, int precision, const CoopOpts& opts,
                             void* workspace, int64_t workspace_bytes, hipStream_t s) {
    bool pre = nets.pregates[0] != nullptr;
    for (int n = 0; n < n_nets; ++n)
        if ((nets.pregates[n] != nullptr) != pre)
            GNNPN_FAIL(GNNPN_E_ARG, "lstm_encode: all nets of a call must use the same input-side form");
    const int prec = precision;
    const int abl = (gnnpn_option_lstm_ablate() & ~(0x800 | 0x1000 | 0x2000)) | (opts.write_through ? 128 : 0);
    const bool diag = (abl & ~128) != 0;
    if (diag && (prec == 1 || pre || (prec == 2 && (abl & ~(128 | 32)) != 0)))
        GNNPN_FAIL(GNNPN_E_UNSUP, "lstm_encode: diagnostics are built for the folded form (fp32: all switches; split: stamps only)");
    CoopLaunch c;
    if (const int rc = coop_begin("lstm_encode", n_nets, B, encode_workspace_bytes, GNNPN_STATUS_ENC_EXPECTED, opts, workspace,
                                  workspace_bytes, s, c))
        return rc;
    u64* p_x = reinterpret_cast<u64*>(c.buffers);
    const int abl_arg = abl | (opts.paired_start ? 0x1000 : 0);
    static unsigned* p_diag = gnnpn_decode_diag_buffer();
#define GNNPN_ENC(PREC_, PRE_, DIAG_)                                                                                        \
    hipLaunchKernelGGL((lstm_encode_coop_kernel<PREC_, PRE_, DIAG_>), dim3(COOP_OVERSUB * c.groups * G), dim3(256),             \
                       gnnpn_lds_padding((const void*)lstm_encode_coop_kernel<PREC_, PRE_, DIAG_>, opts.lds_kb), s, nets, p_x, \
                       c.status, opts.sticky, B, L, n_nets, c.groups_per_net, c.gpx, abl_arg, c.seats, p_diag)
    if (diag) {
        if (prec == 2) GNNPN_ENC(2, false, true);
        else GNNPN_ENC(0, false, true);
    } else if (prec == 2 && pre) GNNPN_ENC(2, true, false);
    else if (prec == 2) GNNPN_ENC(2, false, false);
    else if (prec == 1 && pre) GNNPN_ENC(1, true, false);
    else if (prec == 1) GNNPN_ENC(1, false, false);
    else if (pre) GNNPN_ENC(0, true, false);
    else GNNPN_ENC(0, false, false);
#undef GNNPN_ENC
    return GNNPN_OK;
}
```

gnnpn-sc_amd/csrc/lstm_shared.h:

```cpp
#pragma once
#include "common.h"

#define GNNPN_MAX_NETS 4

struct LstmNets {
    const float* pregates[GNNPN_MAX_NETS];
    const float* inputs[GNNPN_MAX_NETS];
    const float* w_in[GNNPN_MAX_NETS];
    const float* b_in[GNNPN_MAX_NETS];
    const float* whh[GNNPN_MAX_NETS];
    const void* whh_split[GNNPN_MAX_NETS];
    const float* bhh[GNNPN_MAX_NETS];
    float* enc_out[GNNPN_MAX_NETS];
    float* h_n[GNNPN_MAX_NETS];
    float* c_n[GNNPN_MAX_NETS];
};


struct CoopOpts {
    int impl = 0, lds_kb = 0;
    bool write_through = false, paired_start = false;
    unsigned* sticky = nullptr;
};
inline CoopOpts coop_opts(const gnnpn_launch_opts_t* o) {
    CoopOpts c;
    if (o) {
        c.impl = o->impl;
        c.lds_kb = o->lds_kb;
        c.write_through = o->write_through != 0;
        c.paired_start = o->paired_start != 0;
        c.sticky = o->sticky_status;
    }
    return c;
}

int gnnpn_launch_encode_coop(const LstmNets& nets, int n_nets, int32_t B, int32_t L, int precision, const CoopOpts& opts,
                             void* workspace, int64_t workspace_bytes, hipStream_t s);
constexpr int COOP_SEAT_TABLE_WORDS = 8 * 256 + 8 + 8;
unsigned* gnnpn_cu_seat_table();
extern thread_local int64_t g_gnnpn_last_units;
int gnnpn_option_lstm_ablate();
```

gnnpn-sc_amd/csrc/split_probe.hip:

```cpp
#include "common.h"
#include "coop_common.h"

namespace {
constexpr int H = 256;

__global__ __launch_bounds__(256) void split3_pieces_kernel(const float* __restrict__ x, int64_t n, int scale_log2,
                                                           uint16_t* __restrict__ p0, uint16_t* __restrict__ p1,
                                                           uint16_t* __restrict__ p2) {
    const int64_t i = blockIdx.x * (int64_t)blockDim.x + threadIdx.x;
    if (i >= n) return;
    _Float16 a, b, c;
    split3(__fmul_rn(x[i], ldexpf(1.0f, scale_log2)), a, b, c);
    p0[i] = f16_bits(a);
    p1[i] = f16_bits(b);
    p2[i] = f16_bits(c);
}

template <bool SPLIT>
__global__ __launch_bounds__(256) void recurrent_product_kernel(const float* __restrict__ Wp, const float* __restrict__ h,
                                                                float* __restrict__ gates, float* __restrict__ col_inv) {
    __shared__ __attribute__((aligned(16))) float hs[3 * SPLIT_TILE / 2];
    __shared__ __attribute__((aligned(16))) unsigned wts[SPLIT ? SPLIT_WT_DWORDS : 4];
    const int tid = threadIdx.x, lane = tid & 63, wave = tid >> 6, kq = lane >> 4, c = lane & 15;
    const int member = blockIdx.x;
    const int unit = member * 32 + wave * 8 + (c & 7);
    int wrow[2] = {(0 + (c >> 3)) * H + unit, (2 + (c >> 3)) * H + unit};
    f32x4 acc[2] = {f32x4{0.f, 0.f, 0.f, 0.f}, f32x4{0.f, 0.f, 0.f, 0.f}};
    if constexpr (SPLIT) {
        f16x8 w0[2][8], w1[2][8];
        float inv[2];
        unsigned* wt_lane = wts + (wave * 8 * 64 + lane) * 4;
        for (int tl = 0; tl < 2; ++tl) {
            inv[tl] = split_weights<H>(Wp, wrow[tl] / H, wrow[tl] % H, kq, w0[tl], w1[tl], wt_lane + 2 * tl);
            if (kq == 0) col_inv[wrow[tl]] = inv[tl];
        }
        for (int j = 0; j < 16; ++j) split_store(reinterpret_cast<_Float16*>(hs) + j * LDH16 + tid, h[j * H + tid]);
        __syncthreads();
        split_chain(reinterpret_cast<const _Float16*>(hs) + c * LDH16 + 8 * kq, w0, w1, wt_lane, inv, acc);
    } else {
        float wB[2][64];
        for (int tl = 0; tl < 2; ++tl)
            for (int kk = 0; kk < 64; ++kk)
                wB[tl][kk] = Wp[((size_t)(kk * 4 + wrow[tl] / H) * H + wrow[tl] % H) * 4 + kq];
        for (int j = 0; j < 16; ++j) hs[ht_index(j, tid)] = h[j * H + tid];
        __syncthreads();
        mfma_chain_pair<LDT, 16, true>(hs, c, kq, wB[0], wB[1], acc[0], acc[1]);
    }
    for (int tl = 0; tl < 2; ++tl)
        for (int r = 0; r < 4; ++r) gates[(size_t)(4 * kq + r) * (4 * H) + wrow[tl]] = acc[tl][r];
}
}

extern "C" int gnnpn_split3_pieces_f32(const float* x, int64_t n, int32_t scale_log2, uint16_t* p0, uint16_t* p1, uint16_t* p2,
                                       void* stream) {
    GNNPN_REQUIRE(x && p0 && p1 && p2 && n >= 0 && scale_log2 >= -126 && scale_log2 <= 126, "split3_pieces: bad arguments");
    if (n == 0) return GNNPN_OK;
    hipLaunchKernelGGL(split3_pieces_kernel, dim3((unsigned)((n + 255) / 256)), dim3(256), 0, static_cast<hipStream_t>(stream), x, n,
                       (int)scale_log2, p0, p1, p2);
    GNNPN_CHECK_LAUNCH("split3_pieces_f32");
    return GNNPN_OK;
}

extern "C" int gnnpn_recurrent_product_f32(const float* whh_packed, const float* h, int32_t precision, float* gates,
                                           float* col_inv, void* stream) {
    GNNPN_REQUIRE(whh_packed && h && gates, "recurrent_product: null operand");
    GNNPN_REQUIRE(precision == GNNPN_PREC_F32 || precision == GNNPN_PREC_SPLIT, "recurrent_product: precision must be GNNPN_PREC_F32 or GNNPN_PREC_SPLIT");
    hipStream_t s = static_cast<hipStream_t>(stream);
    if (precision == GNNPN_PREC_SPLIT) {
        GNNPN_REQUIRE(col_inv != nullptr, "recurrent_product: col_inv [4H] required for the split precision");
        hipLaunchKernelGGL(recurrent_product_kernel<true>, dim3(8), dim3(256), 0, s, whh_packed, h, gates, col_inv);
    } else {
        hipLaunchKernelGGL(recurrent_product_kernel<false>, dim3(8), dim3(256), 0, s, whh_packed, h, gates, col_inv);
    }
    GNNPN_CHECK_LAUNCH("recurrent_product_f32");
    return GNNPN_OK;
}

namespace {
__global__ __launch_bounds__(256) void lds_interferer_kernel(unsigned ticks, unsigned* __restrict__ sink) {
    extern __shared__ unsigned held[];
    held[threadIdx.x] = threadIdx.x;
    const unsigned long long t0 = __builtin_amdgcn_s_memrealtime();
    while (__builtin_amdgcn_s_memrealtime() - t0 < ticks) __builtin_amdgcn_s_sleep(16);
    if (held[threadIdx.x] == 0xFFFFFFFFu && sink) *sink = 1u;
}
}

extern "C" int gnnpn_debug_lds_interferer(int32_t n_workgroups, int32_t lds_bytes, int32_t hold_us, void* stream) {
    GNNPN_REQUIRE(n_workgroups > 0 && n_workgroups <= 4096 && lds_bytes >= 1024 && lds_bytes <= 160 * 1024 && hold_us >= 0 && hold_us <= 100000,
                  "debug_lds_interferer: bad arguments");
    if (hipFuncSetAttribute((const void*)lds_interferer_kernel, hipFuncAttributeMaxDynamicSharedMemorySize, lds_bytes) != hipSuccess)
        GNNPN_FAIL(GNNPN_E_LAUNCH, "debug_lds_interferer: cannot reserve %d B of LDS", lds_bytes);
    hipLaunchKernelGGL(lds_interferer_kernel, dim3((unsigned)n_workgroups), dim3(256), (unsigned)lds_bytes, static_cast<hipStream_t>(stream),
                       (unsigned)hold_us * 100u, static_cast<unsigned*>(nullptr));
    GNNPN_CHECK_LAUNCH("debug_lds_interferer");
    return GNNPN_OK;
}

namespace {
typedef _Float16 dbg_f16x8 __attribute__((ext_vector_type(8)));
typedef float dbg_f32x4 __attribute__((ext_vector_type(4)));
__global__ __launch_bounds__(64) void debug_mfma_f16_kernel(const float* __restrict__ A, const float* __restrict__ B,
                                                            const float* __restrict__ C, float* __restrict__ D) {
    const int lane = threadIdx.x, c = lane & 15, kq = lane >> 4;
    dbg_f32x4 acc;
    for (int r = 0; r < 4; ++r) acc[r] = C[(4 * kq + r) * 16 + c];
    dbg_f16x8 a, b;
    for (int j = 0; j < 8; ++j) {
        a[j] = (_Float16)A[c * 32 + 8 * kq + j];
        b[j] = (_Float16)B[(8 * kq + j) * 16 + c];
    }
    acc = __builtin_amdgcn_mfma_f32_16x16x32_f16(a, b, acc, 0, 0, 0);
    for (int r = 0; r < 4; ++r) D[(4 * kq + r) * 16 + c] = acc[r];
}
}

extern "C" int gnnpn_debug_mfma_f16(const float* A, const float* B, const float* C, float* D, void* stream) {
    GNNPN_REQUIRE(A && B && C && D, "debug_mfma_f16: null operand");
    hipLaunchKernelGGL(debug_mfma_f16_kernel, dim3(1), dim3(64), 0, static_cast<hipStream_t>(stream), A, B, C, D);
    GNNPN_CHECK_LAUNCH("debug_mfma_f16");
    return GNNPN_OK;
}
```

Before: 477,200.

## Pre-expand leading third-piece weight blocks in LDS to skip per-step perm unpacking

The third f16 piece of each split recurrent weight is normally kept in LDS as packed bytes and unpacked with v_perm on every step of the split MFMA chain. The first few k-blocks are now stored already expanded to f16 in LDS, so the chain reads them straight into MFMA operands and skips the perm instructions for those blocks. This is on by default for the encoder (4 blocks) and the decoder (2 blocks), selected by a runtime flag that picks between two template instantiations. It costs more LDS per workgroup (checked against a 78 KB budget), extra LDS read traffic, and changes to the encoder loop padding nops.

```diff
diff --git a/gnnpn-sc_amd/csrc/api.hip b/gnnpn-sc_amd/csrc/api.hip
--- a/gnnpn-sc_amd/csrc/api.hip
+++ b/gnnpn-sc_amd/csrc/api.hip
@@ -23,6 +23,8 @@
 
 static int g_lstm_ablate = 0;
 int gnnpn_option_lstm_ablate() { return g_lstm_ablate; }
+static int g_split_expanded = GNNPN_SPLIT_EXPANDED_DEFAULT;
+int gnnpn_option_split_expanded() { return g_split_expanded; }
 
 unsigned* gnnpn_cu_seat_table() {
     static unsigned* table[64] = {nullptr};
@@ -60,6 +62,11 @@
     if (!strcmp(name, "lstm_ablate")) {
         GNNPN_REQUIRE(value >= 0 && (value & 128) == 0, "set_option: lstm_ablate bit 7 is gnnpn_launch_opts_t.write_through now");
         g_lstm_ablate = value;
+        return GNNPN_OK;
+    }
+    if (!strcmp(name, "split_expanded")) {
+        GNNPN_REQUIRE(value >= -1 && value <= 3, "set_option: split_expanded is 0..3 (bit 0 encoder, bit 1 decoder), or -1 for the default");
+        g_split_expanded = value < 0 ? GNNPN_SPLIT_EXPANDED_DEFAULT : value;
         return GNNPN_OK;
     }
     GNNPN_FAIL(GNNPN_E_ARG, "set_option: unknown option '%s' (impl / lds_kb / write_through are gnnpn_launch_opts_t fields)", name);
diff --git a/gnnpn-sc_amd/csrc/coop_common.h b/gnnpn-sc_amd/csrc/coop_common.h
--- a/gnnpn-sc_amd/csrc/coop_common.h
+++ b/gnnpn-sc_amd/csrc/coop_common.h
@@ -380,10 +380,21 @@
     at[2 * SPLIT_TILE] = p2;
 }
 
-constexpr int SPLIT_WT_DWORDS = 4 * 8 * 64 * 4;
+constexpr int COOP_SPLIT_LDS_KB = 78;
+#ifndef GNNPN_SPLIT_EXPANDED_DEFAULT
+#define GNNPN_SPLIT_EXPANDED_DEFAULT 3
+#endif
+constexpr int split_wt_dwords(int nexp) { return 4 * (8 + nexp) * 64 * 4; }
+constexpr int SPLIT_WT_DWORDS = split_wt_dwords(0);
+__device__ __forceinline__ unsigned* split_wt_lane(unsigned* wts, int wave, int lane, int nexp) { return wts + (wave * (8 + nexp) * 64 + lane) * 4; }
+__device__ __forceinline__ f16x8 split_expand(unsigned lo, unsigned hi) {
+    const u32x4 r = {__builtin_amdgcn_perm(0u, lo, 0x010c000cu), __builtin_amdgcn_perm(0u, lo, 0x030c020cu),
+                     __builtin_amdgcn_perm(0u, hi, 0x010c000cu), __builtin_amdgcn_perm(0u, hi, 0x030c020cu)};
+    return __builtin_bit_cast(f16x8, r);
+}
 template <int HD>
 __device__ __forceinline__ float split_weights(const float* __restrict__ Wp, int gate, int u, int kq, f16x8 (&w0)[8],
-                                               f16x8 (&w1)[8], unsigned* wt) {
+                                               f16x8 (&w1)[8], unsigned* wt, int tl, int nexp = 0) {
     float m = 0.0f;
 #pragma unroll
     for (int kk = 0; kk < 8; ++kk)
@@ -409,15 +420,19 @@
             w1[kk][j] = p1;
             bytes[j >> 2] |= (unsigned)(f16_bits(p2) >> 8) << (8 * (j & 3));
         }
-        wt[4 * 64 * kk] = bytes[0];
-        wt[4 * 64 * kk + 1] = bytes[1];
+        if (kk < nexp) {
+            *reinterpret_cast<f16x8*>(wt + 4 * 64 * (2 * kk + tl)) = split_expand(bytes[0], bytes[1]);
+        } else {
+            wt[4 * 64 * (nexp + kk) + 2 * tl] = bytes[0];
+            wt[4 * 64 * (nexp + kk) + 2 * tl + 1] = bytes[1];
+        }
     }
     return ldexpf(1.0f, -(15 + s));
 }
 constexpr int SPLIT_PACK_U4_PER_MEMBER = 2 * 2 * 8 * 256 + 8 * 256 + 2 * 256 / 4;
 constexpr int SPLIT_PACK_MEMBERS = 8;
 __device__ __forceinline__ void load_split_weights(const uint4* __restrict__ pk, int tid, f16x8 (&w0)[2][8], f16x8 (&w1)[2][8],
-                                                   unsigned* wt_lane, float (&inv)[2]) {
+                                                   unsigned* wt_lane, float (&inv)[2], int nexp = 0) {
 #pragma unroll
     for (int tl = 0; tl < 2; ++tl)
 #pragma unroll
@@ -426,18 +441,21 @@
             w1[tl][kk] = __builtin_bit_cast(f16x8, pk[((tl * 2 + 1) * 8 + kk) * 256 + tid]);
         }
 #pragma unroll
-    for (int kk = 0; kk < 8; ++kk) *reinterpret_cast<uint4*>(wt_lane + 4 * 64 * kk) = pk[8192 + kk * 256 + tid];
+    for (int kk = 0; kk < 8; ++kk) {
+        const uint4 b = pk[8192 + kk * 256 + tid];
+        if (kk < nexp) {
+            *reinterpret_cast<f16x8*>(wt_lane + 4 * 64 * (2 * kk)) = split_expand(b.x, b.y);
+            *reinterpret_cast<f16x8*>(wt_lane + 4 * 64 * (2 * kk + 1)) = split_expand(b.z, b.w);
+        } else {
+            *reinterpret_cast<uint4*>(wt_lane + 4 * 64 * (nexp + kk)) = b;
+        }
+    }
     const float* fi = reinterpret_cast<const float*>(pk + 10240);
     inv[0] = fi[tid];
     inv[1] = fi[256 + tid];
 }
 
-__device__ __forceinline__ f16x8 split_expand(unsigned lo, unsigned hi) {
-    const u32x4 r = {__builtin_amdgcn_perm(0u, lo, 0x010c000cu), __builtin_amdgcn_perm(0u, lo, 0x030c020cu),
-                     __builtin_amdgcn_perm(0u, hi, 0x010c000cu), __builtin_amdgcn_perm(0u, hi, 0x030c020cu)};
-    return __builtin_bit_cast(f16x8, r);
-}
-template <typename Mid = NoHook>
+template <int NEXP = 0, typename Mid = NoHook>
 __device__ __forceinline__ void split_chain(const _Float16* base, const f16x8 (&w0)[2][8], const f16x8 (&w1)[2][8],
                                             const unsigned* wt, const float (&inv)[2], f32x4 (&acc)[2], Mid mid = Mid()) {
     constexpr int NT = 2;
@@ -449,32 +467,52 @@
     f16x8 h1 = *reinterpret_cast<const f16x8*>(base + SPLIT_TILE);
     f16x8 h2 = *reinterpret_cast<const f16x8*>(base + 2 * SPLIT_TILE);
     u32x4 t = *reinterpret_cast<const u32x4*>(wt);
+    u32x4 x1 = {0u, 0u, 0u, 0u};
+    if constexpr (NEXP > 0) x1 = *reinterpret_cast<const u32x4*>(wt + 4 * 64);
 #define GNNPN_FENCE __builtin_amdgcn_sched_barrier(0)
 #pragma unroll
     for (int kk = 0; kk < 8; ++kk) {
         const int nx = 32 * (kk + 1), cur = kk & 1;
+        const bool bytes = NEXP == 0 || kk >= NEXP;
         u32x4 e0, e1;
+        if (NEXP > 0 && !bytes) {
+            e0 = t;
+            e1 = x1;
+        }
         if (kk < 7) h0[cur ^ 1] = *reinterpret_cast<const f16x8*>(base + nx);
         GNNPN_FENCE;
         a2[0] = __builtin_amdgcn_mfma_f32_16x16x32_f16(h1, w1[0][kk], a2[0], 0, 0, 0);
-        e0.x = __builtin_amdgcn_perm(0u, t.x, 0x010c000cu);
-        e0.y = __builtin_amdgcn_perm(0u, t.x, 0x030c020cu);
+        if (NEXP == 0 || bytes) {
+            e0.x = __builtin_amdgcn_perm(0u, t.x, 0x010c000cu);
+            e0.y = __builtin_amdgcn_perm(0u, t.x, 0x030c020cu);
+        }
         GNNPN_FENCE;
         a2[1] = __builtin_amdgcn_mfma_f32_16x16x32_f16(h1, w1[1][kk], a2[1], 0, 0, 0);
-        e0.z = __builtin_amdgcn_perm(0u, t.y, 0x010c000cu);
-        e0.w = __builtin_amdgcn_perm(0u, t.y, 0x030c020cu);
+        if (NEXP == 0 || bytes) {
+            e0.z = __builtin_amdgcn_perm(0u, t.y, 0x010c000cu);
+            e0.w = __builtin_amdgcn_perm(0u, t.y, 0x030c020cu);
+        }
         GNNPN_FENCE;
         a1[0] = __builtin_amdgcn_mfma_f32_16x16x32_f16(h1, w0[0][kk], a1[0], 0, 0, 0);
-        e1.x = __builtin_amdgcn_perm(0u, t.z, 0x010c000cu);
-        e1.y = __builtin_amdgcn_perm(0u, t.z, 0x030c020cu);
+        if (NEXP == 0 || bytes) {
+            e1.x = __builtin_amdgcn_perm(0u, t.z, 0x010c000cu);
+            e1.y = __builtin_amdgcn_perm(0u, t.z, 0x030c020cu);
+        }
         GNNPN_FENCE;
         a1[1] = __builtin_amdgcn_mfma_f32_16x16x32_f16(h1, w0[1][kk], a1[1], 0, 0, 0);
-        e1.z = __builtin_amdgcn_perm(0u, t.w, 0x010c000cu);
-        e1.w = __builtin_amdgcn_perm(0u, t.w, 0x030c020cu);
+        if (NEXP == 0 || bytes) {
+            e1.z = __builtin_amdgcn_perm(0u, t.w, 0x010c000cu);
+            e1.w = __builtin_amdgcn_perm(0u, t.w, 0x030c020cu);
+        }
         GNNPN_FENCE;
         if (kk < 7) {
             h1 = *reinterpret_cast<const f16x8*>(base + SPLIT_TILE + nx);
-            t = *reinterpret_cast<const u32x4*>(wt + 4 * 64 * (kk + 1));
+            if (NEXP > 0 && kk + 1 < NEXP) {
+                t = *reinterpret_cast<const u32x4*>(wt + 4 * 64 * (2 * kk + 2));
+                x1 = *reinterpret_cast<const u32x4*>(wt + 4 * 64 * (2 * kk + 3));
+            } else {
+                t = *reinterpret_cast<const u32x4*>(wt + 4 * 64 * (NEXP + kk + 1));
+            }
         }
         a2[0] = __builtin_amdgcn_mfma_f32_16x16x32_f16(h0[cur], __builtin_bit_cast(f16x8, e0), a2[0], 0, 0, 0);
         GNNPN_FENCE;
diff --git a/gnnpn-sc_amd/csrc/decode_lean.hip b/gnnpn-sc_amd/csrc/decode_lean.hip
--- a/gnnpn-sc_amd/csrc/decode_lean.hip
+++ b/gnnpn-sc_amd/csrc/decode_lean.hip
@@ -12,6 +12,12 @@
 constexpr int KW = 16;
 constexpr unsigned SPIN_LIMIT = 400000;
 constexpr int XP_GRANULES = ROWS * KW * G;
+#ifndef GNNPN_DEC_NEXP
+#define GNNPN_DEC_NEXP 2
+#endif
+constexpr int DEC_NEXP = GNNPN_DEC_NEXP;
+constexpr int lean_split_lds_bytes(int nexp) { return 3 * SPLIT_TILE * 2 + split_wt_dwords(nexp) * 4 + ROWS * (UNITS + 4) * 4 + ROWS * KW * 8 * 4 + ROWS * 4 + 16; }
+static_assert(lean_split_lds_bytes(DEC_NEXP) <= COOP_SPLIT_LDS_KB * 1024, "the expanded blocks must fit the common footprint");
 
 typedef unsigned u32x2 __attribute__((ext_vector_type(2)));
 constexpr int AUX_SC1 = 16;
@@ -52,19 +58,14 @@
 }
 }
 
-template <bool SPLIT, int OCC, int EVH, bool DIAG = false>
-__global__ __launch_bounds__(256, OCC) void pointer_decode_lean_kernel(DecodeArgs a, u64* xh, u64* xp,
-                                                                     u64* xl, unsigned* __restrict__ err,
-                                                                     unsigned* __restrict__ sticky, int n_nets, int groups_per_net,
-                                                                     int gpx, int write_through, unsigned* __restrict__ seats,
-                                                                     unsigned* __restrict__ diag) {
-    __shared__ __attribute__((aligned(16))) float hs[SPLIT ? 3 * SPLIT_TILE / 2 : ROWS * LDT];
-    __shared__ __attribute__((aligned(16))) unsigned wts[SPLIT ? SPLIT_WT_DWORDS : 4];
-    __shared__ __attribute__((aligned(16))) float hsl[ROWS][UNITS + 4];
-    __shared__ __attribute__((aligned(16))) float win[ROWS][KW][8];
-    __shared__ int sel[ROWS];
-    __shared__ int abort_flag;
-    __shared__ int place[2];
+template <bool SPLIT, int OCC, int EVH, bool DIAG, int NX>
+__device__ __forceinline__ void pointer_decode_lean_body(const DecodeArgs& a, u64* xh, u64* xp, u64* xl, unsigned* __restrict__ err,
+                                                         unsigned* __restrict__ sticky, int n_nets, int groups_per_net, int gpx,
+                                                         int write_through, unsigned* __restrict__ seats, unsigned* __restrict__ diag,
+                                                         float* hs, unsigned* wts, float (*hsl)[UNITS + 4], float (*win)[KW][8],
+                                                         int* sel, int& abort_flag, int* place) {
+    static_assert(SPLIT || NX == 0, "only the exact-split builds keep third pieces");
+    constexpr int nexp = NX;
 
     const int tid = threadIdx.x, lane = tid & 63, wave = __builtin_amdgcn_readfirstlane(tid >> 6);
     const int kq = lane >> 4, c = lane & 15;
@@ -92,18 +93,18 @@
     float wBh[SPLIT ? 1 : 2][SPLIT ? 1 : 64];
     f16x8 wH16[SPLIT ? 2 : 1][8], wL16[SPLIT ? 2 : 1][8];
     float winv[2] = {1.0f, 1.0f};
-    unsigned* wt_lane = wts + (SPLIT ? (wave * 8 * 64 + lane) * 4 : 0);
+    unsigned* wt_lane = SPLIT ? split_wt_lane(wts, wave, lane, nexp) : wts;
     float bh[2], bi[2], sg[2], wXf[2][2];
     const uint4* __restrict__ Wsplit = SPLIT ? static_cast<const uint4*>(net.whh_split) : nullptr;
     if constexpr (SPLIT) {
-        if (Wsplit) load_split_weights(Wsplit + (size_t)member * SPLIT_PACK_U4_PER_MEMBER, tid, wH16, wL16, wt_lane, winv);
+        if (Wsplit) load_split_weights(Wsplit + (size_t)member * SPLIT_PACK_U4_PER_MEMBER, tid, wH16, wL16, wt_lane, winv, nexp);
     }
 #pragma unroll
     for (int tl = 0; tl < 2; ++tl) {
         const int wrow = tl ? wrow1 : wrow0, gate = wrow / H, u = wrow % H;
         bh[tl] = net.bhh[wrow];
         if constexpr (SPLIT) {
-            if (!Wsplit) winv[tl] = split_weights<H>(net.whh, gate, u, kq, wH16[tl], wL16[tl], wt_lane + 2 * tl);
+            if (!Wsplit) winv[tl] = split_weights<H>(net.whh, gate, u, kq, wH16[tl], wL16[tl], wt_lane, tl, nexp);
         } else {
 #pragma unroll
             for (int kk = 0; kk < 64; ++kk) wBh[tl][kk] = net.whh[((size_t)(kk * 4 + gate) * H + u) * 4 + kq];
@@ -253,7 +254,10 @@
                             vl = __builtin_amdgcn_raw_buffer_load_b64(r_lat, vo_lat, (unsigned)(((k - 1) * ROWS + wave * 4) * K) * 8u, AUX_SC1);
                     }
                 };
-                if constexpr (SPLIT) split_chain(reinterpret_cast<const _Float16*>(hs) + c * LDH16 + 8 * kq, wH16, wL16, wt_lane, winv, ah, request_p);
+                if constexpr (SPLIT) {
+                    const _Float16* hbase = reinterpret_cast<const _Float16*>(hs) + c * LDH16 + 8 * kq;
+                    split_chain<NX>(hbase, wH16, wL16, wt_lane, winv, ah, request_p);
+                }
                 else mfma_chain_pair<LDT, OCC == 2 ? 8 : 16, true>(hs, c, kq, wBh[0], wBh[SPLIT ? 0 : 1], ah[0], ah[1], request_p);
                 if constexpr (DIAG) {
                     asm volatile("" ::"v"(ah[0][0]), "v"(ah[1][0]));
@@ -435,6 +439,26 @@
         if (abort_flag) coop_raise(err, sticky, 2u, seats);
         coop_note_finished(sticky, GNNPN_STATUS_DEC_FINISHED, tiles_done);
     }
+}
+
+template <bool SPLIT, int OCC, int EVH, bool DIAG = false>
+__global__ __launch_bounds__(256, OCC) void pointer_decode_lean_kernel(DecodeArgs a, u64* xh, u64* xp,
+                                                                     u64* xl, unsigned* __restrict__ err,
+                                                                     unsigned* __restrict__ sticky, int n_nets, int groups_per_net,
+                                                                     int gpx, int write_through, unsigned* __restrict__ seats,
+                                                                     unsigned* __restrict__ diag) {
+    constexpr int NEXP = SPLIT ? DEC_NEXP : 0;
+    __shared__ __attribute__((aligned(16))) float hs[SPLIT ? 3 * SPLIT_TILE / 2 : ROWS * LDT];
+    __shared__ __attribute__((aligned(16))) unsigned wts[SPLIT ? split_wt_dwords(NEXP) : 4];
+    __shared__ __attribute__((aligned(16))) float hsl[ROWS][UNITS + 4];
+    __shared__ __attribute__((aligned(16))) float win[ROWS][KW][8];
+    __shared__ int sel[ROWS];
+    __shared__ int abort_flag;
+    __shared__ int place[2];
+    if (NEXP > 0 && (write_through & 4))
+        pointer_decode_lean_body<SPLIT, OCC, EVH, DIAG, NEXP>(a, xh, xp, xl, err, sticky, n_nets, groups_per_net, gpx, write_through, seats, diag, hs, wts, hsl, win, sel, abort_flag, place);
+    else
+        pointer_decode_lean_body<SPLIT, OCC, EVH, DIAG, 0>(a, xh, xp, xl, err, sticky, n_nets, groups_per_net, gpx, write_through, seats, diag, hs, wts, hsl, win, sel, abort_flag, place);
 }
 
 struct PickProbArgs {
@@ -490,6 +514,10 @@
     const bool wide = args.K > 8;
     const bool stamps = (gnnpn_option_lstm_ablate() & 0x800) != 0;
     if (stamps && wide) GNNPN_FAIL(GNNPN_E_UNSUP, "pointer_decode: the stamped build exists for n_per <= 8");
+    const bool expanded = split && DEC_NEXP > 0 && (gnnpn_option_split_expanded() & 2) != 0;
+    if (split && opts.lds_kb > 0 && opts.lds_kb * 1024 < lean_split_lds_bytes(DEC_NEXP))
+        GNNPN_FAIL(GNNPN_E_ARG, "pointer_decode: opts.lds_kb = %d is below the %d B of LDS the exact-split kernel holds", opts.lds_kb,
+                   lean_split_lds_bytes(DEC_NEXP));
     CoopLaunch c;
     const auto need = [&](int groups) { return lean_workspace(groups, args.B, args.T, args.K).total(); };
     if (const int rc = coop_begin("pointer_decode", n_nets, args.B, need, GNNPN_STATUS_DEC_EXPECTED, opts, workspace, workspace_bytes, s, c))
@@ -499,7 +527,7 @@
     u64* p_p = reinterpret_cast<u64*>(c.buffers + w.h_bytes);
     u64* p_l = reinterpret_cast<u64*>(c.buffers + w.h_bytes + w.p_bytes);
     static unsigned* p_diag = gnnpn_decode_diag_buffer();
-    const int wt = (opts.write_through ? 1 : 0) | (opts.paired_start ? 2 : 0);
+    const int wt = (opts.write_through ? 1 : 0) | (opts.paired_start ? 2 : 0) | (expanded ? 4 : 0);
 #define GNNPN_LEAN(SPLIT_, OCC_, EVH_, ...)                                                                                           \
     hipLaunchKernelGGL((pointer_decode_lean_kernel<SPLIT_, OCC_, EVH_, ##__VA_ARGS__>), dim3(COOP_OVERSUB * c.groups * G), dim3(256),       \
                        gnnpn_lds_padding((const void*)pointer_decode_lean_kernel<SPLIT_, OCC_, EVH_, ##__VA_ARGS__>, opts.lds_kb), s, args, \
diff --git a/gnnpn-sc_amd/csrc/lstm_coop.hip b/gnnpn-sc_amd/csrc/lstm_coop.hip
--- a/gnnpn-sc_amd/csrc/lstm_coop.hip
+++ b/gnnpn-sc_amd/csrc/lstm_coop.hip
@@ -11,7 +11,13 @@
 constexpr int UNITS = H / G;
 constexpr unsigned SPIN_LIMIT = 400000;
 constexpr int GROUP_GRANULES = 2 * ROWS * H + 2 * 4 * G;
-constexpr int ENC_LOOP_PAD_NOPS = 13;
+#ifndef GNNPN_ENC_NEXP
+#define GNNPN_ENC_NEXP 4
+#endif
+constexpr int ENC_NEXP = GNNPN_ENC_NEXP;
+constexpr int enc_split_lds_bytes(int nexp) { return 3 * SPLIT_TILE * 2 + ROWS * UNITS * 4 + split_wt_dwords(nexp) * 4 + 16; }
+static_assert(enc_split_lds_bytes(ENC_NEXP) <= COOP_SPLIT_LDS_KB * 1024, "the expanded blocks must fit the common footprint");
+constexpr int enc_loop_pad_nops(bool pre, int nexp) { return nexp ? (pre ? 12 : 20) : (pre ? 12 : 19); }
 }
 
 template <int PREC>
@@ -61,22 +67,18 @@
 }
 
 
-template <int PREC, bool PRE, bool DIAG>
-__global__ __launch_bounds__(256, 2) void lstm_encode_coop_kernel(LstmNets nets, u64* __restrict__ xchg,
-                                                                  unsigned* __restrict__ err, unsigned* __restrict__ sticky,
-                                                                  int32_t B, int32_t L, int n_nets, int groups_per_net,
-                                                                  int gpx, int ablate_arg, unsigned* __restrict__ seats,
-                                                                  unsigned* __restrict__ diag) {
-    const int ablate = DIAG ? (ablate_arg & ~0x1000) : (ablate_arg & 128);
+template <int PREC, bool PRE, bool DIAG, int NX>
+__device__ __forceinline__ void lstm_encode_coop_body(const LstmNets& nets, u64* __restrict__ xchg, unsigned* __restrict__ err,
+                                                      unsigned* __restrict__ sticky, int32_t B, int32_t L, int n_nets,
+                                                      int groups_per_net, int gpx, int ablate_arg, unsigned* __restrict__ seats,
+                                                      unsigned* __restrict__ diag, float* hs, float (*hst)[UNITS], int& abort_flag,
+                                                      int* place, unsigned* wts) {
+    const int ablate = DIAG ? (ablate_arg & ~(0x1000 | 0x4000)) : (ablate_arg & 128);
     constexpr bool F16 = PREC != 0, SPLIT = PREC == 2;
     constexpr int HS_FLOATS = PREC == 2 ? 3 * SPLIT_TILE / 2 : ROWS * LDH16;
-    __shared__ __attribute__((aligned(16))) float hs[HS_FLOATS];
-    __shared__ __attribute__((aligned(16))) float hst[ROWS][UNITS];
-    __shared__ int abort_flag;
 
     const int lane = threadIdx.x & 63, wave = threadIdx.x >> 6;
     const int kq = lane >> 4, c = lane & 15;
-    __shared__ int place[2];
     int group, member;
     u64 p_entry = 0, p_placed = 0, p_weights = 0;
     if constexpr (DIAG) p_entry = phase_stamp();
@@ -103,18 +105,19 @@
     f16x8 wB16[F16 ? 2 : 1][8];
     f16x8 wL16[SPLIT ? 2 : 1][8];
     float winv[2] = {1.0f, 1.0f};
-    __shared__ __attribute__((aligned(16))) unsigned wts[SPLIT ? SPLIT_WT_DWORDS : 4];
-    unsigned* wt_lane = wts + (SPLIT ? (wave * 8 * 64 + lane) * 4 : 0);
+    static_assert(SPLIT || NX == 0, "only the exact-split builds keep third pieces");
+    constexpr int nexp = NX;
+    unsigned* wt_lane = SPLIT ? split_wt_lane(wts, wave, lane, nexp) : wts;
     const uint4* __restrict__ Wsplit = SPLIT ? static_cast<const uint4*>(nets.whh_split[net]) : nullptr;
     if constexpr (SPLIT) {
-        if (Wsplit) load_split_weights(Wsplit + (size_t)member * SPLIT_PACK_U4_PER_MEMBER, threadIdx.x, wB16, wL16, wt_lane, winv);
+        if (Wsplit) load_split_weights(Wsplit + (size_t)member * SPLIT_PACK_U4_PER_MEMBER, threadIdx.x, wB16, wL16, wt_lane, winv, nexp);
     }
 #pragma unroll
     for (int tl = 0; tl < 2; ++tl) {
         const int gate = wrow[tl] / H, u = wrow[tl] % H;
         bh[tl] = nets.bhh[net][wrow[tl]];
         if constexpr (SPLIT) {
-            if (!Wsplit) winv[tl] = split_weights<H>(Wp, gate, u, kq, wB16[tl], wL16[tl], wt_lane + 2 * tl);
+            if (!Wsplit) winv[tl] = split_weights<H>(Wp, gate, u, kq, wB16[tl], wL16[tl], wt_lane, tl, nexp);
         } else if constexpr (F16) {
 #pragma unroll
             for (int kk = 0; kk < 8; ++kk)
@@ -165,7 +168,7 @@
         };
         load_input(0, pg_next, ax_next);
 #ifndef GNNPN_ENC_PAD_NOPS
-#define GNNPN_ENC_PAD_NOPS ENC_LOOP_PAD_NOPS
+#define GNNPN_ENC_PAD_NOPS enc_loop_pad_nops(PRE, NX)
 #endif
         if constexpr (SPLIT && !DIAG) asm volatile(".p2align 6\n\t.rept %0\n\ts_nop 0\n\t.endr" ::"n"(GNNPN_ENC_PAD_NOPS) : "memory");
         for (int t = 0; t < L; ++t, ++step) {
@@ -223,7 +226,8 @@
             if constexpr (SPLIT) {
                 if (t > 0) {
                     f32x4 acc[2] = {acc0, acc1};
-                    split_chain(reinterpret_cast<const _Float16*>(hs) + c * LDH16 + 8 * kq, wB16, wL16, wt_lane, winv, acc);
+                    const _Float16* hbase = reinterpret_cast<const _Float16*>(hs) + c * LDH16 + 8 * kq;
+                    split_chain<NX>(hbase, wB16, wL16, wt_lane, winv, acc);
                     acc0 = acc[0];
                     acc1 = acc[1];
                 }
@@ -338,6 +342,26 @@
 }
 
 
+template <int PREC, bool PRE, bool DIAG>
+__global__ __launch_bounds__(256, 2) void lstm_encode_coop_kernel(LstmNets nets, u64* __restrict__ xchg,
+                                                                  unsigned* __restrict__ err, unsigned* __restrict__ sticky,
+                                                                  int32_t B, int32_t L, int n_nets, int groups_per_net,
+                                                                  int gpx, int ablate_arg, unsigned* __restrict__ seats,
+                                                                  unsigned* __restrict__ diag) {
+    constexpr int NEXP = PREC == 2 ? ENC_NEXP : 0;
+    constexpr int HS_FLOATS = PREC == 2 ? 3 * SPLIT_TILE / 2 : ROWS * LDH16;
+    __shared__ __attribute__((aligned(16))) float hs[HS_FLOATS];
+    __shared__ __attribute__((aligned(16))) float hst[ROWS][UNITS];
+    __shared__ __attribute__((aligned(16))) unsigned wts[PREC == 2 ? split_wt_dwords(NEXP) : 4];
+    __shared__ int abort_flag;
+    __shared__ int place[2];
+    if (NEXP > 0 && (ablate_arg & 0x4000))
+        lstm_encode_coop_body<PREC, PRE, DIAG, NEXP>(nets, xchg, err, sticky, B, L, n_nets, groups_per_net, gpx, ablate_arg, seats, diag, hs, hst, abort_flag, place, wts);
+    else
+        lstm_encode_coop_body<PREC, PRE, DIAG, 0>(nets, xchg, err, sticky, B, L, n_nets, groups_per_net, gpx, ablate_arg, seats, diag, hs, hst, abort_flag, place, wts);
+}
+
+
 __global__ __launch_bounds__(256) void lstm_pack_split_kernel(const float* __restrict__ Wp, uint4* __restrict__ out) {
     __shared__ __attribute__((aligned(16))) unsigned wts[SPLIT_WT_DWORDS];
     const int tid = threadIdx.x, lane = tid & 63, wave = tid >> 6, kq = lane >> 4, c = lane & 15;
@@ -345,9 +369,9 @@
     const int unit = member * UNITS + wave * 8 + (c & 7);
     f16x8 w0[2][8], w1[2][8];
     float inv[2];
-    unsigned* wt_lane = wts + (wave * 8 * 64 + lane) * 4;
-#pragma unroll
-    for (int tl = 0; tl < 2; ++tl) inv[tl] = split_weights<H>(Wp, 2 * tl + (c >> 3), unit, kq, w0[tl], w1[tl], wt_lane + 2 * tl);
+    unsigned* wt_lane = split_wt_lane(wts, wave, lane, 0);
+#pragma unroll
+    for (int tl = 0; tl < 2; ++tl) inv[tl] = split_weights<H>(Wp, 2 * tl + (c >> 3), unit, kq, w0[tl], w1[tl], wt_lane, tl);
     uint4* pk = out + (size_t)member * SPLIT_PACK_U4_PER_MEMBER;
 #pragma unroll
     for (int tl = 0; tl < 2; ++tl)
@@ -388,16 +412,20 @@
         if ((nets.pregates[n] != nullptr) != pre)
             GNNPN_FAIL(GNNPN_E_ARG, "lstm_encode: all nets of a call must use the same input-side form");
     const int prec = precision;
-    const int abl = (gnnpn_option_lstm_ablate() & ~(0x800 | 0x1000 | 0x2000)) | (opts.write_through ? 128 : 0);
+    const int abl = (gnnpn_option_lstm_ablate() & ~(0x800 | 0x1000 | 0x2000 | 0x4000)) | (opts.write_through ? 128 : 0);
     const bool diag = (abl & ~128) != 0;
     if (diag && (prec == 1 || pre || (prec == 2 && (abl & ~(128 | 32)) != 0)))
         GNNPN_FAIL(GNNPN_E_UNSUP, "lstm_encode: diagnostics are built for the folded form (fp32: all switches; split: stamps only)");
+    const bool expanded = prec == 2 && ENC_NEXP > 0 && (gnnpn_option_split_expanded() & 1) != 0;
+    if (prec == 2 && opts.lds_kb > 0 && opts.lds_kb * 1024 < enc_split_lds_bytes(ENC_NEXP))
+        GNNPN_FAIL(GNNPN_E_ARG, "lstm_encode: opts.lds_kb = %d is below the %d B of LDS the exact-split kernel holds", opts.lds_kb,
+                   enc_split_lds_bytes(ENC_NEXP));
     CoopLaunch c;
     if (const int rc = coop_begin("lstm_encode", n_nets, B, encode_workspace_bytes, GNNPN_STATUS_ENC_EXPECTED, opts, workspace,
                                   workspace_bytes, s, c))
         return rc;
     u64* p_x = reinterpret_cast<u64*>(c.buffers);
-    const int abl_arg = abl | (opts.paired_start ? 0x1000 : 0);
+    const int abl_arg = abl | (opts.paired_start ? 0x1000 : 0) | (expanded ? 0x4000 : 0);
     static unsigned* p_diag = gnnpn_decode_diag_buffer();
 #define GNNPN_ENC(PREC_, PRE_, DIAG_)                                                                                        \
     hipLaunchKernelGGL((lstm_encode_coop_kernel<PREC_, PRE_, DIAG_>), dim3(COOP_OVERSUB * c.groups * G), dim3(256),             \
diff --git a/gnnpn-sc_amd/csrc/lstm_shared.h b/gnnpn-sc_amd/csrc/lstm_shared.h
--- a/gnnpn-sc_amd/csrc/lstm_shared.h
+++ b/gnnpn-sc_amd/csrc/lstm_shared.h
@@ -40,3 +40,4 @@
 unsigned* gnnpn_cu_seat_table();
 extern thread_local int64_t g_gnnpn_last_units;
 int gnnpn_option_lstm_ablate();
+int gnnpn_option_split_expanded();
diff --git a/gnnpn-sc_amd/csrc/split_probe.hip b/gnnpn-sc_amd/csrc/split_probe.hip
--- a/gnnpn-sc_amd/csrc/split_probe.hip
+++ b/gnnpn-sc_amd/csrc/split_probe.hip
@@ -31,7 +31,7 @@
         float inv[2];
         unsigned* wt_lane = wts + (wave * 8 * 64 + lane) * 4;
         for (int tl = 0; tl < 2; ++tl) {
-            inv[tl] = split_weights<H>(Wp, wrow[tl] / H, wrow[tl] % H, kq, w0[tl], w1[tl], wt_lane + 2 * tl);
+            inv[tl] = split_weights<H>(Wp, wrow[tl] / H, wrow[tl] % H, kq, w0[tl], w1[tl], wt_lane, tl);
             if (kq == 0) col_inv[wrow[tl]] = inv[tl];
         }
         for (int j = 0; j < 16; ++j) split_store(reinterpret_cast<_Float16*>(hs) + j * LDH16 + tid, h[j * H + tid]);
```

Result: no change. 481,300, median of 6 (+0.9%).
